# HiLab-git/FPL-plus

Hardware: AMD Instinct MI355X
Metric: 3D volumes/sec (train step, 80x160x160) (higher is better)
Workload: dtype bf16; 1 GPU; UNet3D-DSBN 32-base-ch bf16 (fp32 master weights), per-GPU batch 2x1x80x160x160 synthetic VS crops, DiceLoss + Adam, domain alternating per step; global_batch=2, parallelism=dp1, step=zero_grad+forward+loss+backward+allreduce+adam

## Files before the change

### fpl-plus_amd/csrc/common.h

```cpp
#pragma once
#include <hip/hip_runtime.h>
#include <math.h>
#include <stdint.h>
#include <stdio.h>
#include <stdarg.h>
#include <string.h>
#include "../../include/fplx.h"

typedef __bf16 bf16_t;

#define FPLX_WAVE 64

inline char* fplx_err_buf() {
  static thread_local char buf[512];
  return buf;
}
inline int fplx_fail(int code, const char* fmt, ...) {
  va_list ap;
  va_start(ap, fmt);
  vsnprintf(fplx_err_buf(), 512, fmt, ap);
  va_end(ap);
  return code;
}
inline int fplx_check_launch(const char* what) {
  hipError_t e = hipGetLastError();
  if (e != hipSuccess) return fplx_fail(FPLX_E_HIP, "%s: %s", what, hipGetErrorString(e));
  return FPLX_OK;
}
#define FPLX_REQUIRE(cond, code, ...) \
  do {                                 \
    if (!(cond)) return fplx_fail(code, __VA_ARGS__); \
  } while (0)

template <typename T> struct Act;
template <> struct Act<float> {
  static __device__ __forceinline__ float ld(const float* p) { return *p; }
  static __device__ __forceinline__ void st(float* p, float v) { *p = v; }
};
template <> struct Act<bf16_t> {
  static __device__ __forceinline__ float ld(const bf16_t* p) { return (float)*p; }
  static __device__ __forceinline__ void st(bf16_t* p, float v) { *p = (bf16_t)v; }
};

__device__ __forceinline__ float ld_dt(const void* p, int64_t i, int dt) {
  return dt == FPLX_F32 ? ((const float*)p)[i] : (float)((const bf16_t*)p)[i];
}
__device__ __forceinline__ void st_dt(void* p, int64_t i, int dt, float v) {
  if (dt == FPLX_F32) ((float*)p)[i] = v;
  else ((bf16_t*)p)[i] = (bf16_t)v;
}

__device__ __forceinline__ uint32_t key_nan_high(float f) {
  if (f != f) return 0xFFFFFFFFu;
  const uint32_t u = __float_as_uint(f);
  return (u & 0x80000000u) ? ~u : (u | 0x80000000u);
}
__device__ __forceinline__ uint32_t key_nan_low(float f) {
  if (f != f) return 0u;
  const uint32_t u = __float_as_uint(f);
  return (u & 0x80000000u) ? ~u : (u | 0x80000000u);
}
__device__ __forceinline__ float key_to_float(uint32_t k) {
  return __uint_as_float((k & 0x80000000u) ? (k & 0x7FFFFFFFu) : ~k);
}

__device__ __forceinline__ float wave_sum(float v) {
#pragma unroll
  for (int o = 32; o > 0; o >>= 1) v += __shfl_xor(v, o, 64);
  return v;
}
__device__ __forceinline__ double wave_sum_d(double v) {
#pragma unroll
  for (int o = 32; o > 0; o >>= 1) v += __shfl_xor(v, o, 64);
  return v;
}

#ifdef __HIPCC__
struct FplxOptimConst { float lr, wd, gscale, k0, k1, k2, k3, k4, k5; int first; };
__device__ __forceinline__ float fplx_optim_grad(float pi, float g, const FplxOptimConst& c) {
  return fmaf(c.wd, pi, g * c.gscale);
}
__device__ __forceinline__ void fplx_adam_elem(float& pi, float g, float& mi, float& vi, const FplxOptimConst& c) {
  const float gi = fplx_optim_grad(pi, g, c);
  mi = fmaf(c.k0, mi, c.k1 * gi);
  vi = fmaf(c.k3, vi, (c.k4 * gi) * gi);
  const float denom = fmaf(sqrtf(vi), c.k5, c.k2);
  pi = fmaf(-c.lr, mi / denom, pi);
}
template <bool MOM>
__device__ __forceinline__ void fplx_sgd_elem(float& pi, float g, float& buf, const FplxOptimConst& c) {
  const float gi = fplx_optim_grad(pi, g, c);
  if (MOM) {
    buf = fmaf(c.k0, buf, gi);
    pi = fmaf(-c.lr, buf, pi);
  } else {
    pi = fmaf(-c.lr, gi, pi);
  }
}
__device__ __forceinline__ void fplx_adadelta_elem(float& pi, float g, float& sq, float& acc, const FplxOptimConst& c) {
  const float gi = fplx_optim_grad(pi, g, c);
  sq = fmaf(c.k0, sq, (c.k1 * gi) * gi);
  const float stdv = sqrtf(sq + c.k2);
  const float ratio = sqrtf(acc + c.k2) / stdv;
  const float delta = ratio * gi;
  acc = fmaf(c.k0, acc, (c.k1 * delta) * delta);
  pi = fmaf(-c.lr, delta, pi);
}
__device__ __forceinline__ void fplx_adagrad_elem(float& pi, float g, float& sum, const FplxOptimConst& c) {
  const float gi = fplx_optim_grad(pi, g, c);
  sum = fmaf(gi, gi, sum);
  const float stdv = sqrtf(sum) + c.k2;
  pi = fmaf(-c.lr, gi / stdv, pi);
}
__device__ __forceinline__ void fplx_adamax_elem(float& pi, float g, float& mi, float& ui, const FplxOptimConst& c) {
  const float gi = fplx_optim_grad(pi, g, c);
  mi = fmaf(c.k0, mi, c.k1 * gi);
  const float decayed = c.k3 * ui;
  ui = fmaxf(decayed, fabsf(gi) + c.k2);
  pi = fmaf(-c.lr, mi / ui, pi);
}
__device__ __forceinline__ void fplx_asgd_elem(float& pi, float g, float& ax, const FplxOptimConst& c) {
  const float gi = fplx_optim_grad(pi, g, c);
  const float decayed = pi * c.k0;
  pi = fmaf(-c.lr, gi, decayed);
  const float d = pi - ax;
  ax = c.k3 == 1.f ? pi : fmaf(d, c.k3, ax);
}
template <bool MOM>
__device__ __forceinline__ void fplx_rmsprop_elem(float& pi, float g, float& sq, float& buf, const FplxOptimConst& c) {
  const float gi = fplx_optim_grad(pi, g, c);
  sq = fmaf(c.k0, sq, (c.k1 * gi) * gi);
  const float avg = sqrtf(sq) + c.k2;
  if (MOM) {
    buf = fmaf(c.k3, buf, gi / avg);
    pi = fmaf(-c.lr, buf, pi);
  } else {
    pi = fmaf(-c.lr, gi / avg, pi);
  }
}
__device__ __forceinline__ void fplx_rprop_elem(float& pi, float g, float& prev, float& ss, const FplxOptimConst& c) {
  float gi = g * c.gscale;
  if (c.first) { prev = 0.f; ss = c.lr; }
  const float s = gi * prev;
  const float f = s > 0.f ? c.k1 : (s < 0.f ? c.k0 : 1.f);
  const float scaled = ss * f;
  ss = fminf(fmaxf(scaled, c.k3), c.k4);
  if (s < 0.f) gi = 0.f;
  const float sg = gi > 0.f ? 1.f : (gi < 0.f ? -1.f : 0.f);
  pi = fmaf(-sg, ss, pi);
  prev = gi;
}
template <int KIND, int NS>
__device__ __forceinline__ void fplx_optim_elem(float& pi, float g, float& s0, float& s1, const FplxOptimConst& c) {
  if constexpr (KIND == FPLX_OPT_SGD) fplx_sgd_elem<NS == 1>(pi, g, s0, c);
  else if constexpr (KIND == FPLX_OPT_ADADELTA) fplx_adadelta_elem(pi, g, s0, s1, c);
  else if constexpr (KIND == FPLX_OPT_ADAGRAD) fplx_adagrad_elem(pi, g, s0, c);
  else if constexpr (KIND == FPLX_OPT_ADAMAX) fplx_adamax_elem(pi, g, s0, s1, c);
  else if constexpr (KIND == FPLX_OPT_ASGD) fplx_asgd_elem(pi, g, s0, c);
  else if constexpr (KIND == FPLX_OPT_RMSPROP) fplx_rmsprop_elem<NS == 2>(pi, g, s0, s1, c);
  else if constexpr (KIND == FPLX_OPT_ADAM) fplx_adam_elem(pi, g, s0, s1, c);
  else fplx_rprop_elem(pi, g, s0, s1, c);
}
#define FPLX_OPTIM_DISPATCH(kind, ns, X)                                       \
  switch ((kind) * 4 + (ns)) {                                                 \
    case FPLX_OPT_SGD * 4 + 0: X(FPLX_OPT_SGD, 0); break;                      \
    case FPLX_OPT_SGD * 4 + 1: X(FPLX_OPT_SGD, 1); break;                      \
    case FPLX_OPT_ADADELTA * 4 + 2: X(FPLX_OPT_ADADELTA, 2); break;            \
    case FPLX_OPT_ADAGRAD * 4 + 1: X(FPLX_OPT_ADAGRAD, 1); break;              \
    case FPLX_OPT_ADAMAX * 4 + 2: X(FPLX_OPT_ADAMAX, 2); break;                \
    case FPLX_OPT_ASGD * 4 + 1: X(FPLX_OPT_ASGD, 1); break;                    \
    case FPLX_OPT_RMSPROP * 4 + 1: X(FPLX_OPT_RMSPROP, 1); break;              \
    case FPLX_OPT_RMSPROP * 4 + 2: X(FPLX_OPT_RMSPROP, 2); break;              \
    case FPLX_OPT_ADAM * 4 + 2: X(FPLX_OPT_ADAM, 2); break;                    \
    default: X(FPLX_OPT_RPROP, 2); break;                                      \
  }
static inline int fplx_optim_consts(const char* who, int kind, const float* hp, int nhp, int step, float gscale, const void* s0,
                                    const void* s1, FplxOptimConst* c, int* ns) {
  static const int want[FPLX_OPT_COUNT] = {3, 4, 4, 5, 4, 5, 5, 5};
  FPLX_REQUIRE(kind >= 0 && kind < FPLX_OPT_COUNT, FPLX_E_BADSHAPE, "%s: unknown optimiser kind %d (0..%d)", who, kind,
               FPLX_OPT_COUNT - 1);
  FPLX_REQUIRE(hp, FPLX_E_NULL, "%s: null hyper-parameter array", who);
  FPLX_REQUIRE(nhp == want[kind], FPLX_E_BADSHAPE, "%s: kind %d takes %d hyper-parameters, got %d", who, kind, want[kind], nhp);
  FPLX_REQUIRE(step >= 1, FPLX_E_BADSHAPE, "%s: step=%d (1-based)", who, step);
  *c = {hp[0], 0.f, gscale, 0.f, 0.f, 0.f, 0.f, 0.f, 0.f, step == 1};
  int need = 2;
  switch (kind) {
    case FPLX_OPT_SGD:
      c->k0 = hp[1]; c->wd = hp[2];
      need = hp[1] != 0.f ? 1 : 0;
      break;
    case FPLX_OPT_ADADELTA:
      c->k0 = hp[1]; c->k1 = (float)(1.0 - (double)hp[1]); c->k2 = hp[2]; c->wd = hp[3];
      break;
    case FPLX_OPT_ADAGRAD:
      c->lr = (float)((double)hp[0] / (1.0 + (double)(step - 1) * (double)hp[1])); c->k2 = hp[2]; c->wd = hp[3];
      need = 1;
      break;
    case FPLX_OPT_ADAMAX:
      c->lr = (float)((double)hp[0] / (1.0 - pow((double)hp[1], step)));
      c->k0 = hp[1]; c->k1 = (float)(1.0 - (double)hp[1]); c->k3 = hp[2]; c->k2 = hp[3]; c->wd = hp[4];
      break;
    case FPLX_OPT_ASGD:
      c->k0 = (float)(1.0 - (double)hp[2] * (double)hp[0]); c->k3 = hp[1]; c->wd = hp[3];
      need = 1;
      break;
    case FPLX_OPT_RMSPROP:
      c->k0 = hp[1]; c->k1 = (float)(1.0 - (double)hp[1]); c->k2 = hp[2]; c->k3 = hp[3]; c->wd = hp[4];
      need = hp[3] > 0.f ? 2 : 1;
      break;
    case FPLX_OPT_ADAM:
      c->lr = (float)((double)hp[0] / (1.0 - pow((double)hp[1], step)));
      c->k0 = hp[1]; c->k1 = 1.f - hp[1]; c->k2 = hp[3]; c->k3 = hp[2]; c->k4 = 1.f - hp[2]; c->wd = hp[4];
      c->k5 = (float)(1.0 / sqrt(1.0 - pow((double)hp[2], step)));
      break;
    default:
      c->k0 = hp[1]; c->k1 = hp[2]; c->k3 = hp[3]; c->k4 = hp[4];
      break;
  }
  FPLX_REQUIRE((need < 1 || s0) && (need < 2 || s1), FPLX_E_NULL, "%s: kind %d needs %d state buffer(s) here", who, kind, need);
  *ns = need;
  return FPLX_OK;
}
struct FplxBlock { int x, y, z; };
__device__ __forceinline__ FplxBlock fplx_xcd_block(int on) {
  FplxBlock b = {(int)blockIdx.x, (int)blockIdx.y, (int)blockIdx.z};
  if (!on) return b;
  const unsigned gx = gridDim.x, gy = gridDim.y, gz = gridDim.z, t = gx * gy * gz;
  const unsigned l = (blockIdx.z * gy + blockIdx.y) * gx + blockIdx.x;
  const unsigned xcd = l & 7u, q = t >> 3, r = t & 7u;
  const unsigned lp = xcd * q + (xcd < r ? xcd : r) + (l >> 3);
  const unsigned per = gy * gz, xq = lp / per, rem = lp - xq * per;
  b.x = __builtin_amdgcn_readfirstlane((int)xq);
  b.z = __builtin_amdgcn_readfirstlane((int)(rem / gy));
  b.y = __builtin_amdgcn_readfirstlane((int)(rem % gy));
  return b;
}
struct FplxTileRange { int64_t first, end, step; };
__device__ __forceinline__ FplxTileRange fplx_xcd_tiles(int64_t ntiles, int on) {
  FplxTileRange t = {(int64_t)blockIdx.x, ntiles, (int64_t)gridDim.x};
  if (!on || gridDim.x < 16) return t;
  const unsigned c = blockIdx.x & 7u, xcd = (blockIdx.y * gridDim.x + blockIdx.x) & 7u;
  const int64_t q = ntiles >> 3, r = ntiles & 7;
  const int64_t start = xcd * q + ((int64_t)xcd < r ? xcd : r);
  t.first = start + (blockIdx.x >> 3);
  t.end = start + q + ((int64_t)xcd < r ? 1 : 0);
  t.step = (gridDim.x - c + 7u) >> 3;
  return t;
}
template <typename... P, typename... A>
inline void fplx_launch(void (*kernel)(P...), dim3 grid, dim3 block, size_t lds, hipStream_t st, A... args) {
  if (lds) (void)hipFuncSetAttribute((const void*)kernel, hipFuncAttributeMaxDynamicSharedMemorySize, (int)lds);
  kernel<<<grid, block, lds, st>>>(args...);
}
#endif
#define FPLX_KNOB_LIST(X)                                                                                              \
  X(XCD, "xcd", 1)                                                    \
  X(BRICK, "brick", 1)                                    \
  X(BRICK_FILL, "brick_fill", 192)           \
  X(BRICK_GEO, "brick_geo", -1)                    \
  X(BRICK_KSPLIT, "brick_ksplit", 0)                                             \
  X(EDGE_BLOCKS, "edge_blocks", 1024)                             \
  X(STEM_ROWS, "stem_rows", 1)                                              \
  X(OUTCONV_T, "outconv_t", 1)                                 \
  X(OUTCONV_DGRAD_MFMA, "outconv_dgrad_mfma", 1)                                                                       \
  X(OUTCONV_FWD_ROWS, "outconv_fwd_rows", 1)  \
  X(OUTCONV_DGRAD_ROWS, "outconv_dgrad_rows", 1)  \
  X(PACK_TILED, "pack_tiled", 1)                                                                                       \
  X(PACK_MULTI, "pack_multi", 1)                                                                                       \
  X(MARCH, "march", 1)                           \
  X(MARCH64_FW, "march64_fw", 0)                                \
  X(MARCH_DS, "march_ds", 0)                                       \
  X(MARCH128, "march128", 1)                                                                                           \
  X(MARCH64_LW, "march64_lw", 1)            \
  X(MARCH32_V2, "march32_v2", 4)              \
  X(WG_COT_MINVOX, "wg_cot_minvox", 0)                                                                                 \
  X(WG_TW, "wg_tw", 0)                                                                                                 \
  X(WG_CIT, "wg_cit", 2)                                                                                               \
  X(WG_COT, "wg_cot", 2)                                                                                               \
  X(WG_DS, "wg_ds", 0)                                                                                                 \
  X(WG_VOX, "wg_vox", 1)                              \
  X(WG_ROLL, "wg_roll", 1)                     \
  X(WG_ROLL_GEO, "wg_roll_geo", 0)          \
  X(WG_ROLL_M16, "wg_roll_m16", 1)                 \
  X(WG_ROLL_MB, "wg_roll_mb", 1)            \
  X(WG_ROLL_CUS, "wg_roll_cus", 256)                                \
  X(WG_ROLL_OVH, "wg_roll_ovh", 9)                     \
  X(WG_ROLL_MINVOX, "wg_roll_minvox", 0)                                                   \
  X(WG_ROLL2D, "wg_roll2d", 1)              \
  X(WG_ROLL2D_OVH, "wg_roll2d_ovh", 3)      \
  X(WG_REDUCE_ROWS, "wg_reduce_rows", 8)    \
  X(WG_VOX_LW, "wg_vox_lw", 1)              \
  X(WG_VOX_CUS, "wg_vox_cus", 128)          \
  X(WG_VOX_MAXV, "wg_vox_maxv", 10000)         \
  X(TILE_NT, "tile_nt", 0)                                                                                             \
  X(TILE_KS, "tile_ks", 0)                                                                                             \
  X(MID_TILE, "mid_tile", 1)                                                                                           \
  X(DECONV_ROWS, "deconv_rows", 1)                                                                                     \
  X(DECONV_DGRAD_ROWS, "deconv_dgrad_rows", 1)   \
  X(ROWS_SMALL_DIV, "rows_small_div", 16)   \
  X(EW_GROUP, "ew_group", 1)                                                                                           \
  X(POOL_COL, "pool_col", 1)                         \
  X(EW_INFLIGHT, "ew_inflight", 2)          \
  X(EW_INFLIGHT_REDUCE, "ew_inflight_reduce", 2)
enum FplxKnobId {
#define FPLX_KNOB_ENUM(id, key, def) FPLX_K_##id,
  FPLX_KNOB_LIST(FPLX_KNOB_ENUM)
#undef FPLX_KNOB_ENUM
  FPLX_K_COUNT
};
extern "C" __attribute__((visibility("hidden"))) int64_t fplx_knob_values[FPLX_K_COUNT];
static inline int64_t fplx_knob(int id) { return __atomic_load_n(&fplx_knob_values[id], __ATOMIC_RELAXED); }
static inline int fplx_xcd_on() { return (int)fplx_knob(FPLX_K_XCD); }

static inline int fplx_rows_for(int64_t voxels) {
  constexpr int cap = 512;
  const int div = voxels <= 32768 ? (int)fplx_knob(FPLX_K_ROWS_SMALL_DIV) : 64;
  int64_t r = (voxels + div - 1) / div;
  if (r > cap) r = cap;
  if (r < 1) r = 1;
  return (int)r;
}
```

### fpl-plus_amd/csrc/conv_march.hip

```cpp
#include "internal.h"
#include "gfx950.h"
#include <stdlib.h>
#include <type_traits>

namespace {

__device__ __attribute__((aligned(16))) const unsigned int fplx_zero16[4] = {0u, 0u, 0u, 0u};
#ifdef FPLX_STAMP
__device__ long long* fplx_stamp_buf;
#endif

struct MG {
  static constexpr int CIN = 32, ROWB = 64, CH = 4;
  static constexpr int FH = 16, FW = 32, SH = FH + 2, SW = FW + 2, SLAB = SH * SW;
  static constexpr int THREADS = 512;
  static constexpr int SLAB_CHUNKS = SLAB * CH, SLAB_DMA = (SLAB_CHUNKS + 63) / 64;
  static constexpr int SLAB_BYTES = SLAB_DMA * 1024, W_BYTES = 27 * 32 * ROWB;
  static constexpr int NPIECE = (SLAB_DMA + 7) / 8;
  static constexpr int STAGE_BYTES = 32 * 32 * 2;
  static constexpr int LDS = 2 * SLAB_BYTES + W_BYTES + 32 * 4 + NPIECE * THREADS * 4 + (THREADS / 64) * STAGE_BYTES;
  static __device__ __forceinline__ int swz(int row) { return (row >> 2) & 3; }
};

template <int MASK, class Side>
__device__ __forceinline__ void march_step(const char* __restrict__ sl, const char* __restrict__ wbuf, int wave, int r,
                                           int khalf, f32x16& A00, f32x16& A01, f32x16& A10, f32x16& A11, f32x16& A20,
                                           f32x16& A21, Side&& side) {
  bf16x8 fa[2][2], fb[2][3];
  const f32x16 zero = {0.f, 0.f, 0.f, 0.f, 0.f, 0.f, 0.f, 0.f, 0.f, 0.f, 0.f, 0.f, 0.f, 0.f, 0.f, 0.f};
  int vb = wave * 2 * MG::SW + r, rb = r;
  opaque_v(vb, rb);
  const char* wl0 = wbuf + rb * MG::ROWB + ((khalf ^ MG::swz(rb)) << 4);
  const char* wl1 = wbuf + rb * MG::ROWB + (((2 + khalf) ^ MG::swz(rb)) << 4);
  auto load_stage = [&](int q, int buf) {
    const int p = q >> 1, ks = q & 1;
    const int kh = p / 3, kw = p % 3;
    const int c = 2 * ks + khalf;
#pragma unroll
    for (int m = 0; m < 2; ++m) {
      const int vox = vb + (m + kh) * MG::SW + kw;
      fa[buf][m] = *reinterpret_cast<const bf16x8*>(sl + vox * MG::ROWB + ((c ^ MG::swz(vox)) << 4));
    }
#pragma unroll
    for (int kd = 0; kd < 3; ++kd)
      if ((MASK >> kd) & 1) fb[buf][kd] = *reinterpret_cast<const bf16x8*>((ks ? wl1 : wl0) + (kd * 9 + p) * 32 * MG::ROWB);
  };
  load_stage(0, 0);
#pragma unroll
  for (int q = 0; q < 18; ++q) {
    if (q + 1 < 18) load_stage(q + 1, (q + 1) & 1);
    __builtin_amdgcn_sched_barrier(0);
    const int b = q & 1;
    {
      if constexpr ((MASK & 1) != 0) A00 = __builtin_amdgcn_mfma_f32_32x32x16_bf16(fa[b][0], fb[b][0], q == 0 ? zero : A00, 0, 0, 0);
      if constexpr ((MASK & 2) != 0) A10 = __builtin_amdgcn_mfma_f32_32x32x16_bf16(fa[b][0], fb[b][1], A10, 0, 0, 0);
      if constexpr ((MASK & 4) != 0) A20 = __builtin_amdgcn_mfma_f32_32x32x16_bf16(fa[b][0], fb[b][2], A20, 0, 0, 0);
      if constexpr ((MASK & 1) != 0) A01 = __builtin_amdgcn_mfma_f32_32x32x16_bf16(fa[b][1], fb[b][0], q == 0 ? zero : A01, 0, 0, 0);
      if constexpr ((MASK & 2) != 0) A11 = __builtin_amdgcn_mfma_f32_32x32x16_bf16(fa[b][1], fb[b][1], A11, 0, 0, 0);
      if constexpr ((MASK & 4) != 0) A21 = __builtin_amdgcn_mfma_f32_32x32x16_bf16(fa[b][1], fb[b][2], A21, 0, 0, 0);
    }
    side(q);
    __builtin_amdgcn_sched_barrier(0);
  }
}

template <bool TWOD, bool ACT = false>
__global__ void __launch_bounds__(MG::THREADS)
conv_fwd_march32(const bf16_t* __restrict__ x, int64_t ldx, const bf16_t* __restrict__ wp,
                 const float* __restrict__ bias, bf16_t* __restrict__ y, int64_t ldy, int N, int D, int H, int W,
                 int Cout, float* __restrict__ stats, int tilesH, int tilesW, int dsegs, int dlen,
                 bf16_t* __restrict__ y1, int ysplit, int xcd, const float* __restrict__ slope_p = nullptr) {
  extern __shared__ __attribute__((aligned(16))) char smem[];
#ifdef FPLX_STAMP
  const long long st_launch = __builtin_amdgcn_s_memtime();
#endif
  char* slabs = smem;
  char* wbuf = smem + 2 * MG::SLAB_BYTES;
  float* bias_s = reinterpret_cast<float*>(wbuf + MG::W_BYTES);
  const int tid = threadIdx.x, lane = tid & 63;
  const int wave = __builtin_amdgcn_readfirstlane(tid >> 6);
  const int r = lane & 31, khalf = lane >> 5;
  const FplxBlock bid = fplx_xcd_block(xcd);
  int b = bid.x;
  const int seg = b % dsegs; b /= dsegs;
  const int tw = b % tilesW; b /= tilesW;
  const int th = b % tilesH; b /= tilesH;
  const int n = __builtin_amdgcn_readfirstlane(b);
  const int h0 = __builtin_amdgcn_readfirstlane(th * MG::FH), w0 = __builtin_amdgcn_readfirstlane(tw * MG::FW);
  const int d0 = __builtin_amdgcn_readfirstlane(seg * dlen);
  const int d1 = (d0 + dlen < D) ? d0 + dlen : D;
  const int n0 = bid.y * 32;

  constexpr int NPIECE = MG::NPIECE;
  int* soff_s = reinterpret_cast<int*>(bias_s + 32);
#pragma unroll
  for (int k = 0; k < NPIECE; ++k) {
    const int i = (wave + 8 * k) * 64 + lane;
    const int vox = i >> 2, c = (i & 3) ^ MG::swz(vox);
    const int hh = vox / MG::SW + h0 - 1, ww = vox % MG::SW + w0 - 1;
    const bool in = i < MG::SLAB_CHUNKS && hh >= 0 && hh < H && ww >= 0 && ww < W;
    soff_s[k * MG::THREADS + tid] = in ? (int)((((int64_t)hh * W + ww) * ldx + c * 8) * 2) : -1;
  }
  const int64_t xslice = (int64_t)H * W * ldx * 2;
  const char* xn = reinterpret_cast<const char*>(x) + (int64_t)n * D * xslice;
  auto slab_piece = [&](int s, int k, int so) {
    if (wave + 8 * k < MG::SLAB_DMA) {
      const char* xs = xn + s * xslice;
      const void* src = so >= 0 ? (const void*)(xs + (unsigned)so) : (const void*)fplx_zero16;
      lds_dma_global(src, lds_addr(slabs + ((s + 1) & 1) * MG::SLAB_BYTES + (wave + 8 * k) * 1024));
    }
  };

  f32x16 K0a, K0b, K1a, K1b, K2a, K2b, Ra, Rb;
#pragma unroll
  for (int i = 0; i < 16; ++i) K0a[i] = K0b[i] = K1a[i] = K1b[i] = K2a[i] = K2b[i] = Ra[i] = Rb[i] = 0.f;

  const int sbase = TWOD ? d0 : d0 - 1;
  if (sbase >= 0) {
#pragma unroll
    for (int k = 0; k < NPIECE; ++k) slab_piece(sbase, k, soff_s[k * MG::THREADS + tid]);
  }
  for (int j = wave; j < 27 * 32 * MG::CH / 64; j += 8) {
    const int i = j * 64 + lane;
    const int row = i >> 2, c = (i & 3) ^ MG::swz(row);
    lds_dma_global(wp + ((int64_t)(row >> 5) * Cout + n0 + (row & 31)) * MG::CIN + c * 8, lds_addr(wbuf + j * 1024));
  }
  if (tid < 32) bias_s[tid] = bias ? bias[n0 + tid] : 0.f;
  wait_vmcnt0();
  lds_barrier();

  const float bv = bias_s[r];
  float ssum = 0.f, qsum = 0.f;
  char* stg = reinterpret_cast<char*>(soff_s + NPIECE * MG::THREADS) + wave * MG::STAGE_BYTES;
  char* stg_w = stg + (4 * khalf) * 64 + r * 2;
  const char* stg_r = stg + lane * 16;
  unsigned wmask = 0;
#pragma unroll
  for (int i = 0; i < 16; ++i)
    if (w0 + (i & 3) + 8 * (i >> 2) + 4 * khalf < W) wmask |= 1u << i;
  const bool hok0 = h0 + wave * 2 < H, hok1 = h0 + wave * 2 + 1 < H;
  const unsigned ldy2 = (unsigned)ldy * 2u;
  bf16_t* ysel = bid.y >= ysplit ? y1 + (bid.y - ysplit) * 32 : y + n0;
  char* yn = reinterpret_cast<char*>(ysel) + (((int64_t)n * D * H + (h0 + wave * 2)) * W + w0) * ldy * 2;
  const int64_t yslice = (int64_t)H * W * ldy * 2;
  const unsigned soffb = (unsigned)(lane >> 2) * ldy2 + (unsigned)(lane & 3) * 16u;
  const bool sok0 = w0 + (lane >> 2) < W, sok1 = w0 + (lane >> 2) + 16 < W;
  const float slope_v = ACT ? *slope_p : 0.f;
  auto retire_elem = [&](f32x16& A, int m, int i) {
    const int wu = (i & 3) + 8 * (i >> 2);
    float ov = A[i] + bv;
    if (ACT) ov = ov > 0.f ? ov : ov * slope_v;
    *reinterpret_cast<bf16_t*>(stg_w + wu * 64) = (bf16_t)ov;
#ifndef FPLX_ABL_NOSTATS
    if (!ACT && (m ? hok1 : hok0) && ((wmask >> i) & 1u)) {
      ssum += ov;
      qsum = fmaf(ov, ov, qsum);
    }
#endif
  };
  auto retire_flush = [&](int m, int o) {
    if (m ? hok1 : hok0) {
      unsigned l2 = ldy2;
      opaque_s(l2);
      char* rowp = yn + o * yslice + (unsigned)(m * W) * l2;
      const u32x4 v0 = *reinterpret_cast<const u32x4*>(stg_r);
      const u32x4 v1 = *reinterpret_cast<const u32x4*>(stg_r + 1024);
      if (sok0) global_store_16(rowp + soffb, v0);
      if (sok1) global_store_16(rowp + 16u * l2 + soffb, v1);
    }
  };

  const int nd = d1 - d0;
  const int nsteps = TWOD ? nd + 1 : nd + 2;
#ifdef FPLX_STAMP
  long long st_step = 0, st_wait = 0, st_bar = 0;
  const long long st_begin = __builtin_amdgcn_s_memtime();
  const long long st_rbegin = __builtin_amdgcn_s_memrealtime();
#endif
  for (int t = 0; t < nsteps; ++t) {
#ifdef FPLX_STAMP
    const long long st0 = __builtin_amdgcn_s_memtime();
#endif
    const int s = sbase + t;
    const bool fetch = TWOD ? s + 1 < d1 : (s + 1 <= d1 && s + 1 < D);
    const bool wout = t >= (TWOD ? 2 : 3);
    const int o = s - 2;
    const char* sl = slabs + ((s + 1) & 1) * MG::SLAB_BYTES;
    int so[NPIECE];
#pragma unroll
    for (int k = 0; k < NPIECE; ++k) so[k] = soff_s[k * MG::THREADS + tid];
    auto side = [&](int q) {
#ifndef FPLX_ABL_NODMA
      if (q < NPIECE && fetch) slab_piece(s + 1, q, so[q < NPIECE ? q : 0]);
#endif
#ifdef FPLX_ABL_NORETIRE
      return;
#endif
      if (wout && q < 9) {
        if (q < 4) { retire_elem(Ra, 0, 4 * q); retire_elem(Ra, 0, 4 * q + 1); retire_elem(Ra, 0, 4 * q + 2); retire_elem(Ra, 0, 4 * q + 3); }
        if (q == 4) retire_flush(0, o);
        if (q >= 4 && q < 8) { retire_elem(Rb, 1, 4 * q - 16); retire_elem(Rb, 1, 4 * q - 15); retire_elem(Rb, 1, 4 * q - 14); retire_elem(Rb, 1, 4 * q - 13); }
        if (q == 8) retire_flush(1, o);
      }
    };
#define MARCH_STEP(MASK) march_step<MASK>(sl, wbuf, wave, r, khalf, K0a, K0b, K1a, K1b, K2a, K2b, side)
    if (TWOD ? t < nd : (s >= 0 && s < D)) {
      if constexpr (TWOD) {
        MARCH_STEP(2);
      } else {
        if (t == 0) MARCH_STEP(1);
        else if (t == 1) MARCH_STEP(3);
        else if (t < nd) MARCH_STEP(7);
        else if (t == nd) MARCH_STEP(6);
        else MARCH_STEP(4);
      }
    } else {
#pragma unroll
      for (int q = 0; q < 9; ++q) side(q);
#pragma unroll
      for (int i = 0; i < 16; ++i) K0a[i] = K0b[i] = 0.f;
    }
#undef MARCH_STEP
    Ra = K2a; Rb = K2b; K2a = K1a; K2b = K1b; K1a = K0a; K1b = K0b;
#ifdef FPLX_STAMP
    const long long st1 = __builtin_amdgcn_s_memtime();
#endif
    wait_vmcnt0();
#ifdef FPLX_STAMP
    const long long st2 = __builtin_amdgcn_s_memtime();
#endif
    lds_barrier();
#ifdef FPLX_STAMP
    const long long st3 = __builtin_amdgcn_s_memtime();
    st_step += st1 - st0; st_wait += st2 - st1; st_bar += st3 - st2;
#endif
  }
#ifdef FPLX_STAMP
  if (lane == 0) {
    long long* o = fplx_stamp_buf + ((int64_t)(blockIdx.y * gridDim.x + blockIdx.x) * 8 + wave) * 6;
    o[0] = st_step; o[1] = st_wait; o[2] = st_bar; o[3] = __builtin_amdgcn_s_memtime() - st_begin; o[4] = nsteps;
    o[5] = __builtin_amdgcn_s_memrealtime() - st_rbegin;
  }
#endif
  {
#pragma unroll
    for (int i = 0; i < 16; ++i) retire_elem(Ra, 0, i);
    retire_flush(0, d1 - 1);
#pragma unroll
    for (int i = 0; i < 16; ++i) retire_elem(Rb, 1, i);
    retire_flush(1, d1 - 1);
  }

  if (stats) {
    lds_barrier();
    float* red = reinterpret_cast<float*>(smem);
    const float a = ssum + __shfl_xor(ssum, 32, 64), q2 = qsum + __shfl_xor(qsum, 32, 64);
    if (lane < 32) { red[(wave * 2 + 0) * 32 + r] = a; red[(wave * 2 + 1) * 32 + r] = q2; }
    lds_barrier();
    if (tid < 64) {
      const int which = tid >> 5, c = tid & 31;
      float t = 0.f;
#pragma unroll
      for (int wv = 0; wv < 8; ++wv) t += red[(wv * 2 + which) * 32 + c];
      stats[((int64_t)bid.x * 2 + which) * Cout + n0 + c] = t;
    }
  }
}

struct MG2 {
  static constexpr int CIN = 32, ROWB = 64, CH = 4;
  static constexpr int FH = 16, FW = 32, SH = FH + 2, SW = FW + 2, SLAB = SH * SW;
  static constexpr int THREADS = 256, WAVES = 4;
  static constexpr int SLAB_CHUNKS = SLAB * CH, SLAB_DMA = (SLAB_CHUNKS + 63) / 64;
  static constexpr int SLAB_BYTES = SLAB_DMA * 1024, W_BYTES = 27 * 32 * ROWB;
  static constexpr int NPIECE = (SLAB_DMA + WAVES - 1) / WAVES;
  static constexpr int STAGE_BYTES = 32 * 32 * 2;
  static constexpr int LDS = 2 * SLAB_BYTES + W_BYTES + 32 * 4 + WAVES * 2 * STAGE_BYTES + NPIECE * THREADS * 4;
  static __device__ __forceinline__ int swz(int row) { return (row >> 2) & 3; }
};

template <bool STATS>
__global__ void __launch_bounds__(MG2::THREADS)
conv_fwd_march32v2(const bf16_t* __restrict__ x, int64_t ldx, const bf16_t* __restrict__ wp,
                   const float* __restrict__ bias, bf16_t* __restrict__ y, int64_t ldy, int N, int D, int H, int W,
                   int Cout, float* __restrict__ stats, int tilesH, int tilesW, int dsegs, int dlen,
                   bf16_t* __restrict__ y1, int ysplit, int xcd) {
  using G = MG2;
  extern __shared__ __attribute__((aligned(16))) char smem[];
  char* slabs = smem;
  char* wbuf = smem + 2 * G::SLAB_BYTES;
  float* bias_s = reinterpret_cast<float*>(wbuf + G::W_BYTES);
  const int tid = threadIdx.x, lane = tid & 63;
  const int wave = __builtin_amdgcn_readfirstlane(tid >> 6);
  const int r = lane & 31, khalf = lane >> 5;
  const FplxBlock bid = fplx_xcd_block(xcd);
  int b = bid.x;
  const int seg = b % dsegs; b /= dsegs;
  const int tw = b % tilesW; b /= tilesW;
  const int th = b % tilesH; b /= tilesH;
  const int n = __builtin_amdgcn_readfirstlane(b);
  const int h0 = __builtin_amdgcn_readfirstlane(th * G::FH), w0 = __builtin_amdgcn_readfirstlane(tw * G::FW);
  const int d0 = __builtin_amdgcn_readfirstlane(seg * dlen);
  const int d1 = (d0 + dlen < D) ? d0 + dlen : D;
  const int n0 = bid.y * 32;

  constexpr int NPIECE = G::NPIECE;
  unsigned* voff_s = reinterpret_cast<unsigned*>(smem + 2 * G::SLAB_BYTES + G::W_BYTES + 32 * 4 + G::WAVES * 2 * G::STAGE_BYTES);
#pragma unroll
  for (int k = 0; k < NPIECE; ++k) {
    int piece = wave + G::WAVES * k;
    if (piece > G::SLAB_DMA - 1) piece = G::SLAB_DMA - 1;
    const int i = piece * 64 + lane;
    const int vox = i >> 2, c = (i & 3) ^ G::swz(vox);
    const int hh = vox / G::SW + h0 - 1, ww = vox % G::SW + w0 - 1;
    const bool in = i < G::SLAB_CHUNKS && hh >= 0 && hh < H && ww >= 0 && ww < W;
    voff_s[k * G::THREADS + tid] = in ? (unsigned)((((int64_t)hh * W + ww) * ldx + c * 8) * 2) : 0x40000000u;
  }
  const int64_t xslice = (int64_t)H * W * ldx * 2;
  const char* xn = reinterpret_cast<const char*>(x) + (int64_t)n * D * xslice;
  u32x4 rsrc;
  rsrc[0] = __builtin_amdgcn_readfirstlane((unsigned)(size_t)xn);
  rsrc[1] = __builtin_amdgcn_readfirstlane((unsigned)((size_t)xn >> 32) & 0xFFFFu);
  rsrc[2] = __builtin_amdgcn_readfirstlane((unsigned)((int64_t)D * xslice));
  rsrc[3] = 0x00020000u;
  const unsigned xslice32 = __builtin_amdgcn_readfirstlane((unsigned)xslice);
  auto slab_piece = [&](int s, int k, unsigned vo) {
    int piece = wave + G::WAVES * k;
    if (piece > G::SLAB_DMA - 1) piece = G::SLAB_DMA - 1;
    const unsigned dst = lds_addr(slabs + ((s + 1) & 1) * G::SLAB_BYTES + piece * 1024);
    const unsigned so = __builtin_amdgcn_readfirstlane((s >= 0 && s < D) ? (unsigned)s * xslice32 : 0x40000000u);
    lds_dma_buffer(rsrc, vo, so, dst);
  };

  f32x16 S[4][4];
#pragma unroll
  for (int a = 0; a < 4; ++a)
#pragma unroll
    for (int m = 0; m < 4; ++m)
#pragma unroll
      for (int i = 0; i < 16; ++i) S[a][m][i] = 0.f;

  __syncthreads();
  const int sbase = d0 - 1;
#pragma unroll
  for (int k = 0; k < NPIECE; ++k) slab_piece(sbase, k, voff_s[k * G::THREADS + tid]);
  for (int j = wave; j < 27 * 32 * G::CH / 64; j += G::WAVES) {
    const int i = j * 64 + lane;
    const int row = i >> 2, c = (i & 3) ^ G::swz(row);
    lds_dma_global(wp + ((int64_t)(row >> 5) * Cout + n0 + (row & 31)) * G::CIN + c * 8, lds_addr(wbuf + j * 1024));
  }
  if (tid < 32) bias_s[tid] = bias ? bias[n0 + tid] : 0.f;
  wait_vmcnt0();
  lds_barrier();

  const float bv = bias_s[r];
  float ssum = 0.f, qsum = 0.f;
  char* stg = reinterpret_cast<char*>(bias_s + 32) + wave * 2 * G::STAGE_BYTES;
  const unsigned ldy2 = (unsigned)ldy * 2u;
  bf16_t* ysel = bid.y >= ysplit ? y1 + (bid.y - ysplit) * 32 : y + n0;
  char* yn = reinterpret_cast<char*>(ysel) + (((int64_t)n * D * H + (h0 + wave * 4)) * W + w0) * ldy * 2;
  const int64_t yslice = (int64_t)H * W * ldy * 2;
  const unsigned soffb = (unsigned)(lane >> 2) * ldy2 + (unsigned)(lane & 3) * 16u;
  auto retire_elems = [&](const f32x16& A, int m, int i0, int cnt) {
    char* w_ = stg + (m & 1) * G::STAGE_BYTES + (4 * khalf) * 64 + r * 2;
#pragma unroll
    for (int i = i0; i < i0 + cnt; ++i) {
      const int wu = (i & 3) + 8 * (i >> 2);
      const float ov = A[i] + bv;
      *reinterpret_cast<bf16_t*>(w_ + wu * 64) = (bf16_t)ov;
      if (STATS) { ssum += ov; qsum = fmaf(ov, ov, qsum); }
    }
  };
  auto retire_flush = [&](int m, int o) {
    const char* r_ = stg + (m & 1) * G::STAGE_BYTES + lane * 16;
    unsigned l2 = ldy2;
    opaque_s(l2);
    char* rowp = yn + o * yslice + (unsigned)(m * W) * l2;
    const u32x4 v0 = *reinterpret_cast<const u32x4*>(r_);
    const u32x4 v1 = *reinterpret_cast<const u32x4*>(r_ + 1024);
    global_store_16(rowp + soffb, v0);
    global_store_16(rowp + 16u * l2 + soffb, v1);
  };

  const int nd = d1 - d0;
  const int nsteps = nd + 2;
  const f32x16 zero = {0.f, 0.f, 0.f, 0.f, 0.f, 0.f, 0.f, 0.f, 0.f, 0.f, 0.f, 0.f, 0.f, 0.f, 0.f, 0.f};

  bf16x8 fa[2][6], fb[9];
  auto load_a = [&](const char* sl, int g, int buf) {
    const int kw = g >> 1, ks = g & 1, c = 2 * ks + khalf;
    int vb = wave * 4 * G::SW + r;
    opaque_v(vb);
#pragma unroll
    for (int rho = 0; rho < 6; ++rho) {
      const int vox = vb + rho * G::SW + kw;
      fa[buf][rho] = *reinterpret_cast<const bf16x8*>(sl + vox * G::ROWB + ((c ^ G::swz(vox)) << 4));
    }
  };
  auto load_b = [&](int g, int kd) {
    const int kw = g >> 1, ks = g & 1;
    int rb = r;
    opaque_v(rb);
    const char* wl = wbuf + rb * G::ROWB + (((2 * ks + khalf) ^ G::swz(rb)) << 4);
#pragma unroll
    for (int kh = 0; kh < 3; ++kh)
      fb[kd * 3 + kh] = *reinterpret_cast<const bf16x8*>(wl + ((kd * 9 + kh * 3 + kw) * 32) * G::ROWB);
  };
  load_a(slabs + ((sbase + 1) & 1) * G::SLAB_BYTES, 0, 0);
  load_b(0, 0); load_b(0, 1); load_b(0, 2);
  auto step = [&](auto rot_c, int t) {
    constexpr int ROT = decltype(rot_c)::value;
    const int s = sbase + t;
    const int o = (s - 2 > d0) ? s - 2 : d0;
    const char* sl = slabs + ((s + 1) & 1) * G::SLAB_BYTES;
    const char* sl_next = slabs + (s & 1) * G::SLAB_BYTES;
    const bool on0 = t < nd, on1 = t >= 1 && t <= nd, on2 = t >= 2;
    f32x16 (&K0)[4] = S[(0 - ROT) & 3];
    f32x16 (&K1)[4] = S[(1 - ROT) & 3];
    f32x16 (&K2)[4] = S[(2 - ROT) & 3];
    f32x16 (&R)[4] = S[(3 - ROT) & 3];
    u32x4 fl0, fl1;
    unsigned vo0 = 0, vo1 = 0, vo2 = 0;
#pragma unroll
    for (int g = 0; g < 6; ++g) {
      const int bf = g & 1;
      const int p0 = g < 2 ? 3 * g : 2 * g + 2, np = g < 2 ? 3 : (g < 4 ? 2 : 0);
      if (np > 0) {
        vo0 = voff_s[p0 * G::THREADS + tid];
        vo1 = voff_s[(p0 + 1) * G::THREADS + tid];
        if (np > 2) vo2 = voff_s[(p0 + 2) * G::THREADS + tid];
      }
      if (g >= 1 && g <= 4) {
        const char* r_ = stg + ((g - 1) & 1) * G::STAGE_BYTES + lane * 16;
        fl0 = *reinterpret_cast<const u32x4*>(r_);
        fl1 = *reinterpret_cast<const u32x4*>(r_ + 1024);
      }
      if (g < 4) retire_elems(R[g], g, 0, 8);
      if (on0) {
#pragma unroll
        for (int m = 0; m < 4; ++m)
#pragma unroll
          for (int kh = 0; kh < 3; ++kh)
            K0[m] = __builtin_amdgcn_mfma_f32_32x32x16_bf16(fa[bf][m + kh], fb[0 + kh], (g == 0 && kh == 0) ? zero : K0[m], 0, 0, 0);
      }
      __builtin_amdgcn_sched_barrier(0);
      if (g < 5) load_a(sl, g + 1, bf ^ 1); else load_a(sl_next, 0, 0);
      load_b((g + 1) % 6, 0);
      if (g >= 1 && g <= 4) {
        unsigned l2 = ldy2;
        opaque_s(l2);
        char* rowp = yn + o * yslice + (unsigned)((g - 1) * W) * l2;
        global_store_16(rowp + soffb, fl0);
        global_store_16(rowp + 16u * l2 + soffb, fl1);
      }
      if (np > 0) {
        slab_piece(s + 1, p0, vo0);
        slab_piece(s + 1, p0 + 1, vo1);
        if (np > 2) slab_piece(s + 1, p0 + 2, vo2);
      }
      if (on1) {
#pragma unroll
        for (int m = 0; m < 4; ++m)
#pragma unroll
          for (int kh = 0; kh < 3; ++kh)
            K1[m] = __builtin_amdgcn_mfma_f32_32x32x16_bf16(fa[bf][m + kh], fb[3 + kh], K1[m], 0, 0, 0);
      }
      __builtin_amdgcn_sched_barrier(0);
      load_b((g + 1) % 6, 1);
      if (g < 4) retire_elems(R[g], g, 8, 8);
      if (on2) {
#pragma unroll
        for (int m = 0; m < 4; ++m)
#pragma unroll
          for (int kh = 0; kh < 3; ++kh)
            K2[m] = __builtin_amdgcn_mfma_f32_32x32x16_bf16(fa[bf][m + kh], fb[6 + kh], K2[m], 0, 0, 0);
      }
      load_b((g + 1) % 6, 2);
      __builtin_amdgcn_sched_barrier(0);
      if (g == 4) {
        wait_vmcnt0();
        lds_barrier();
      }
    }
  };
  using C0 = std::integral_constant<int, 0>;
  using C1 = std::integral_constant<int, 1>;
  using C2 = std::integral_constant<int, 2>;
  using C3 = std::integral_constant<int, 3>;
#ifdef FPLX_STAMP
  const long long st_begin = __builtin_amdgcn_s_memtime();
  const long long st_rbegin = __builtin_amdgcn_s_memrealtime();
#endif
  int t = 0;
  for (;;) {
    step(C0{}, t); ++t;
    if (t >= nsteps) break;
    step(C1{}, t); ++t;
    if (t >= nsteps) break;
    step(C2{}, t); ++t;
    if (t >= nsteps) break;
    if (STATS && t == 3) { ssum = 0.f; qsum = 0.f; }
    step(C3{}, t); ++t;
    if (t >= nsteps) break;
  }
#ifdef FPLX_STAMP
  if (lane == 0) {
    long long* o_ = fplx_stamp_buf + ((int64_t)(blockIdx.y * gridDim.x + blockIdx.x) * 8 + wave) * 6;
    o_[0] = 0; o_[1] = 0; o_[2] = 0; o_[3] = __builtin_amdgcn_s_memtime() - st_begin; o_[4] = nsteps;
    o_[5] = __builtin_amdgcn_s_memrealtime() - st_rbegin;
  }
#endif
  auto drain = [&](auto rot_c) {
    constexpr int ROT = decltype(rot_c)::value;
    f32x16 (&R)[4] = S[(3 - ROT) & 3];
#pragma unroll
    for (int m = 0; m < 4; ++m) { retire_elems(R[m], m, 0, 16); retire_flush(m, d1 - 1); }
  };
  switch (nsteps & 3) {
    case 0: drain(C0{}); break;
    case 1: drain(C1{}); break;
    case 2: drain(C2{}); break;
    default: drain(C3{}); break;
  }

  if (STATS && stats) {
    lds_barrier();
    float* red = reinterpret_cast<float*>(smem);
    const float a = ssum + __shfl_xor(ssum, 32, 64), q2 = qsum + __shfl_xor(qsum, 32, 64);
    if (lane < 32) { red[(wave * 2 + 0) * 32 + r] = a; red[(wave * 2 + 1) * 32 + r] = q2; }
    lds_barrier();
    if (tid < 64) {
      const int which = tid >> 5, c = tid & 31;
      float tt = 0.f;
#pragma unroll
      for (int wv = 0; wv < 4; ++wv) tt += red[(wv * 2 + which) * 32 + c];
      stats[((int64_t)bid.x * 2 + which) * Cout + n0 + c] = tt;
    }
  }
}

template <bool STATS, int ASWZ, bool ACT = false>
__global__ void __launch_bounds__(MG2::THREADS)
conv_fwd_march32v3(const bf16_t* __restrict__ x, int64_t ldx, const bf16_t* __restrict__ wp,
                   const float* __restrict__ bias, bf16_t* __restrict__ y, int64_t ldy, int N, int D, int H, int W,
                   int Cout, float* __restrict__ stats, int tilesH, int tilesW, int dsegs, int dlen,
                   bf16_t* __restrict__ y1, int ysplit, int xcd, const float* __restrict__ slope_p = nullptr) {
  using G = MG2;
  extern __shared__ __attribute__((aligned(16))) char smem[];
  char* slabs = smem;
  char* wbuf = smem + 2 * G::SLAB_BYTES;
  float* bias_s = reinterpret_cast<float*>(wbuf + G::W_BYTES);
  const int tid = threadIdx.x, lane = tid & 63;
  const int wave = __builtin_amdgcn_readfirstlane(tid >> 6);
  const int r16 = lane & 15, kg = lane >> 4;
  const FplxBlock bid = fplx_xcd_block(xcd);
  int b = bid.x;
  const int seg = b % dsegs; b /= dsegs;
  const int tw = b % tilesW; b /= tilesW;
  const int th = b % tilesH; b /= tilesH;
  const int n = __builtin_amdgcn_readfirstlane(b);
  const int h0 = __builtin_amdgcn_readfirstlane(th * G::FH), w0 = __builtin_amdgcn_readfirstlane(tw * G::FW);
  const int d0 = __builtin_amdgcn_readfirstlane(seg * dlen);
  const int d1 = (d0 + dlen < D) ? d0 + dlen : D;
  const int n0 = bid.y * 32;

  auto wswz = [](int row) { const int q = (row >> 2) & 3; return (4 - q) & 3; };
  auto aswz = [](int vox) { return ASWZ ? ((vox >> 2) & 1) << 1 : (vox >> 2) & 3; };
  constexpr int NPIECE = G::NPIECE;
  unsigned* voff_s = reinterpret_cast<unsigned*>(smem + 2 * G::SLAB_BYTES + G::W_BYTES + 32 * 4 + G::WAVES * 2 * G::STAGE_BYTES);
#pragma unroll
  for (int k = 0; k < NPIECE; ++k) {
    int piece = wave + G::WAVES * k;
    if (piece > G::SLAB_DMA - 1) piece = G::SLAB_DMA - 1;
    const int i = piece * 64 + lane;
    const int vox = i >> 2, c = (i & 3) ^ aswz(vox);
    const int hh = vox / G::SW + h0 - 1, ww = vox % G::SW + w0 - 1;
    const bool in = i < G::SLAB_CHUNKS && hh >= 0 && hh < H && ww >= 0 && ww < W;
    voff_s[k * G::THREADS + tid] = in ? (unsigned)((((int64_t)hh * W + ww) * ldx + c * 8) * 2) : 0x40000000u;
  }
  const int64_t xslice = (int64_t)H * W * ldx * 2;
  const char* xn = reinterpret_cast<const char*>(x) + (int64_t)n * D * xslice;
  u32x4 rsrc;
  rsrc[0] = __builtin_amdgcn_readfirstlane((unsigned)(size_t)xn);
  rsrc[1] = __builtin_amdgcn_readfirstlane((unsigned)((size_t)xn >> 32) & 0xFFFFu);
  rsrc[2] = __builtin_amdgcn_readfirstlane((unsigned)((int64_t)D * xslice));
  rsrc[3] = 0x00020000u;
  const unsigned xslice32 = __builtin_amdgcn_readfirstlane((unsigned)xslice);
  auto slab_piece = [&](int s, int k, unsigned vo) {
    int piece = wave + G::WAVES * k;
    if (piece > G::SLAB_DMA - 1) piece = G::SLAB_DMA - 1;
    const unsigned dst = lds_addr(slabs + ((s + 1) & 1) * G::SLAB_BYTES + piece * 1024);
    const unsigned so = __builtin_amdgcn_readfirstlane((s >= 0 && s < D) ? (unsigned)s * xslice32 : 0x40000000u);
    lds_dma_buffer(rsrc, vo, so, dst);
  };

  f32x4 S[4][4][4];
#pragma unroll
  for (int a = 0; a < 4; ++a)
#pragma unroll
    for (int m = 0; m < 4; ++m)
#pragma unroll
      for (int q = 0; q < 4; ++q)
#pragma unroll
        for (int i = 0; i < 4; ++i) S[a][m][q][i] = 0.f;

  __syncthreads();
  const int sbase = d0 - 1;
#pragma unroll
  for (int k = 0; k < NPIECE; ++k) slab_piece(sbase, k, voff_s[k * G::THREADS + tid]);
  for (int j = wave; j < 27 * 32 * G::CH / 64; j += G::WAVES) {
    const int i = j * 64 + lane;
    const int row = i >> 2, c = (i & 3) ^ wswz(row);
    lds_dma_global(wp + ((int64_t)(row >> 5) * Cout + n0 + (row & 31)) * G::CIN + c * 8, lds_addr(wbuf + j * 1024));
  }
  if (tid < 32) bias_s[tid] = bias ? bias[n0 + tid] : 0.f;
  wait_vmcnt0();
  lds_barrier();

  const float bv0 = bias_s[r16], bv1 = bias_s[16 + r16];
  float ssum0 = 0.f, qsum0 = 0.f, ssum1 = 0.f, qsum1 = 0.f;
  char* stg = reinterpret_cast<char*>(bias_s + 32) + wave * 2 * G::STAGE_BYTES;
  const unsigned ldy2 = (unsigned)ldy * 2u;
  bf16_t* ysel = bid.y >= ysplit ? y1 + (bid.y - ysplit) * 32 : y + n0;
  char* yn = reinterpret_cast<char*>(ysel) + (((int64_t)n * D * H + (h0 + wave * 4)) * W + w0) * ldy * 2;
  const int64_t yslice = (int64_t)H * W * ldy * 2;
  const unsigned soffb = (unsigned)(lane >> 2) * ldy2 + (unsigned)(lane & 3) * 16u;
  const float slope_v = ACT ? *slope_p : 0.f;
  auto retire_half = [&](const f32x4 (&A)[4], int m, int mh) {
    char* w_ = stg + (m & 1) * G::STAGE_BYTES + (mh * 16 + 4 * kg) * 64 + r16 * 2;
#pragma unroll
    for (int i = 0; i < 4; ++i) {
      float o0 = A[mh * 2 + 0][i] + bv0, o1 = A[mh * 2 + 1][i] + bv1;
      if (ACT) { o0 = o0 > 0.f ? o0 : o0 * slope_v; o1 = o1 > 0.f ? o1 : o1 * slope_v; }
      *reinterpret_cast<bf16_t*>(w_ + i * 64) = (bf16_t)o0;
      *reinterpret_cast<bf16_t*>(w_ + i * 64 + 32) = (bf16_t)o1;
      if (STATS) { ssum0 += o0; qsum0 = fmaf(o0, o0, qsum0); ssum1 += o1; qsum1 = fmaf(o1, o1, qsum1); }
    }
  };
  auto retire_flush = [&](int m, int o) {
    const char* r_ = stg + (m & 1) * G::STAGE_BYTES + lane * 16;
    unsigned l2 = ldy2;
    opaque_s(l2);
    char* rowp = yn + o * yslice + (unsigned)(m * W) * l2;
    const u32x4 v0 = *reinterpret_cast<const u32x4*>(r_);
    const u32x4 v1 = *reinterpret_cast<const u32x4*>(r_ + 1024);
    global_store_16(rowp + soffb, v0);
    global_store_16(rowp + 16u * l2 + soffb, v1);
  };

  const int nd = d1 - d0;
  const int nsteps = nd + 2;
  const f32x4 zero = {0.f, 0.f, 0.f, 0.f};

  bf16x8 fa[2][6], fb[18];
  auto load_a = [&](const char* sl, int g, int buf) {
    const int kw = g >> 1, mh = g & 1;
    int vb = wave * 4 * G::SW + r16;
    opaque_v(vb);
#pragma unroll
    for (int rho = 0; rho < 6; ++rho) {
      const int vox = vb + rho * G::SW + kw + mh * 16;
      fa[buf][rho] = *reinterpret_cast<const bf16x8*>(sl + vox * G::ROWB + ((kg ^ aswz(vox)) << 4));
    }
  };
  auto load_b = [&](int kw, int kd) {
    int rb = r16;
    opaque_v(rb);
    const char* wl = wbuf + rb * G::ROWB + ((kg ^ wswz(rb)) << 4);
#pragma unroll
    for (int kh = 0; kh < 3; ++kh)
#pragma unroll
      for (int nh = 0; nh < 2; ++nh)
        fb[kd * 6 + kh * 2 + nh] = *reinterpret_cast<const bf16x8*>(wl + (((kd * 9 + kh * 3 + kw) * 32) + nh * 16) * G::ROWB);
  };
  load_a(slabs + ((sbase + 1) & 1) * G::SLAB_BYTES, 0, 0);
  load_b(0, 0); load_b(0, 1); load_b(0, 2);
  auto step = [&](auto rot_c, int t) {
    constexpr int ROT = decltype(rot_c)::value;
    const int s = sbase + t;
    const int o = (s - 2 > d0) ? s - 2 : d0;
    const char* sl = slabs + ((s + 1) & 1) * G::SLAB_BYTES;
    const char* sl_next = slabs + (s & 1) * G::SLAB_BYTES;
    const bool on0 = t < nd, on1 = t >= 1 && t <= nd, on2 = t >= 2;
    f32x4 (&K0)[4][4] = S[(0 - ROT) & 3];
    f32x4 (&K1)[4][4] = S[(1 - ROT) & 3];
    f32x4 (&K2)[4][4] = S[(2 - ROT) & 3];
    f32x4 (&R)[4][4] = S[(3 - ROT) & 3];
    u32x4 fl0, fl1;
    unsigned vo0 = 0, vo1 = 0, vo2 = 0;
#pragma unroll
    for (int g = 0; g < 6; ++g) {
      const int bf = g & 1, kw = g >> 1, mh = g & 1;
      const int p0 = g < 2 ? 3 * g : 2 * g + 2, np = g < 2 ? 3 : (g < 4 ? 2 : 0);
      if (np > 0) {
        vo0 = voff_s[p0 * G::THREADS + tid];
        vo1 = voff_s[(p0 + 1) * G::THREADS + tid];
        if (np > 2) vo2 = voff_s[(p0 + 2) * G::THREADS + tid];
      }
      if (g >= 1 && g <= 4) {
        const char* r_ = stg + ((g - 1) & 1) * G::STAGE_BYTES + lane * 16;
        fl0 = *reinterpret_cast<const u32x4*>(r_);
        fl1 = *reinterpret_cast<const u32x4*>(r_ + 1024);
      }
      if (g < 4) retire_half(R[g], g, 0);
      if (on0) {
#pragma unroll
        for (int m = 0; m < 4; ++m)
#pragma unroll
          for (int kh = 0; kh < 3; ++kh)
#pragma unroll
            for (int nh = 0; nh < 2; ++nh)
              K0[m][mh * 2 + nh] = __builtin_amdgcn_mfma_f32_16x16x32_bf16(fa[bf][m + kh], fb[0 + kh * 2 + nh],
                                                                          (kw == 0 && kh == 0) ? zero : K0[m][mh * 2 + nh], 0, 0, 0);
      }
      __builtin_amdgcn_sched_barrier(0);
      if (g < 5) load_a(sl, g + 1, bf ^ 1); else load_a(sl_next, 0, 0);
      if (mh == 1) load_b((kw + 1) % 3, 0);
      if (g >= 1 && g <= 4) {
        unsigned l2 = ldy2;
        opaque_s(l2);
        char* rowp = yn + o * yslice + (unsigned)((g - 1) * W) * l2;
        global_store_16(rowp + soffb, fl0);
        global_store_16(rowp + 16u * l2 + soffb, fl1);
      }
      if (np > 0) {
        slab_piece(s + 1, p0, vo0);
        slab_piece(s + 1, p0 + 1, vo1);
        if (np > 2) slab_piece(s + 1, p0 + 2, vo2);
      }
      if (on1) {
#pragma unroll
        for (int m = 0; m < 4; ++m)
#pragma unroll
          for (int kh = 0; kh < 3; ++kh)
#pragma unroll
            for (int nh = 0; nh < 2; ++nh)
              K1[m][mh * 2 + nh] = __builtin_amdgcn_mfma_f32_16x16x32_bf16(fa[bf][m + kh], fb[6 + kh * 2 + nh], K1[m][mh * 2 + nh], 0, 0, 0);
      }
      __builtin_amdgcn_sched_barrier(0);
      if (mh == 1) load_b((kw + 1) % 3, 1);
      if (g < 4) retire_half(R[g], g, 1);
      if (on2) {
#pragma unroll
        for (int m = 0; m < 4; ++m)
#pragma unroll
          for (int kh = 0; kh < 3; ++kh)
#pragma unroll
            for (int nh = 0; nh < 2; ++nh)
              K2[m][mh * 2 + nh] = __builtin_amdgcn_mfma_f32_16x16x32_bf16(fa[bf][m + kh], fb[12 + kh * 2 + nh], K2[m][mh * 2 + nh], 0, 0, 0);
      }
      if (mh == 1) load_b((kw + 1) % 3, 2);
      __builtin_amdgcn_sched_barrier(0);
      if (g == 4) {
        wait_vmcnt0();
        lds_barrier();
      }
    }
  };
  using C0 = std::integral_constant<int, 0>;
  using C1 = std::integral_constant<int, 1>;
  using C2 = std::integral_constant<int, 2>;
  using C3 = std::integral_constant<int, 3>;
#ifdef FPLX_STAMP
  const long long st_begin = __builtin_amdgcn_s_memtime();
  const long long st_rbegin = __builtin_amdgcn_s_memrealtime();
#endif
  int t = 0;
  for (;;) {
    step(C0{}, t); ++t;
    if (t >= nsteps) break;
    step(C1{}, t); ++t;
    if (t >= nsteps) break;
    step(C2{}, t); ++t;
    if (t >= nsteps) break;
    if (STATS && t == 3) { ssum0 = qsum0 = ssum1 = qsum1 = 0.f; }
    step(C3{}, t); ++t;
    if (t >= nsteps) break;
  }
#ifdef FPLX_STAMP
  if (lane == 0) {
    long long* o_ = fplx_stamp_buf + ((int64_t)(blockIdx.y * gridDim.x + blockIdx.x) * 8 + wave) * 6;
    o_[0] = 0; o_[1] = 0; o_[2] = 0; o_[3] = __builtin_amdgcn_s_memtime() - st_begin; o_[4] = nsteps;
    o_[5] = __builtin_amdgcn_s_memrealtime() - st_rbegin;
  }
#endif
  auto drain = [&](auto rot_c) {
    constexpr int ROT = decltype(rot_c)::value;
    f32x4 (&R)[4][4] = S[(3 - ROT) & 3];
#pragma unroll
    for (int m = 0; m < 4; ++m) { retire_half(R[m], m, 0); retire_half(R[m], m, 1); retire_flush(m, d1 - 1); }
  };
  switch (nsteps & 3) {
    case 0: drain(C0{}); break;
    case 1: drain(C1{}); break;
    case 2: drain(C2{}); break;
    default: drain(C3{}); break;
  }

  if (STATS && stats) {
    lds_barrier();
    float* red = reinterpret_cast<float*>(smem);
    float a0 = ssum0, a1 = ssum1, q0 = qsum0, q1 = qsum1;
    a0 += __shfl_xor(a0, 16, 64); a0 += __shfl_xor(a0, 32, 64);
    a1 += __shfl_xor(a1, 16, 64); a1 += __shfl_xor(a1, 32, 64);
    q0 += __shfl_xor(q0, 16, 64); q0 += __shfl_xor(q0, 32, 64);
    q1 += __shfl_xor(q1, 16, 64); q1 += __shfl_xor(q1, 32, 64);
    if (lane < 16) {
      red[(wave * 2 + 0) * 32 + r16] = a0; red[(wave * 2 + 0) * 32 + 16 + r16] = a1;
      red[(wave * 2 + 1) * 32 + r16] = q0; red[(wave * 2 + 1) * 32 + 16 + r16] = q1;
    }
    lds_barrier();
    if (tid < 64) {
      const int which = tid >> 5, c = tid & 31;
      float tt = 0.f;
#pragma unroll
      for (int wv = 0; wv < 4; ++wv) tt += red[(wv * 2 + which) * 32 + c];
      stats[((int64_t)bid.x * 2 + which) * Cout + n0 + c] = tt;
    }
  }
}

template <int FWV>
struct MG64T {
  static constexpr int ROWB = 64, CH = 4;
  static constexpr int FW = FWV, FH = 256 / FWV, SH = FH + 2, SW = FW + 2, SLAB = SH * SW;
  static constexpr int HPM = 32 / FW;
  static constexpr int THREADS = 256;
  static constexpr int SLAB_CHUNKS = SLAB * CH, SLAB_DMA = (SLAB_CHUNKS + 63) / 64;
  static constexpr int SLAB_BYTES = SLAB * ROWB, WH_BYTES = 27 * 32 * ROWB;
  static constexpr int NPIECE = (SLAB_DMA + 3) / 4;
  static constexpr int STAGE_BYTES = 32 * 32 * 2;
  static constexpr int LDS = 2 * SLAB_BYTES + 2 * WH_BYTES + 32 * 4 + (THREADS / 64) * STAGE_BYTES;
  static __device__ __forceinline__ int swz(int row) { return (row >> 2) & 3; }
};
using MG64 = MG64T<32>;

template <int MASK, bool FIRST, class G, class Side>
__device__ __forceinline__ void march64_half(const char* __restrict__ sl, const char* __restrict__ wh, int wave, int r,
                                             int khalf, f32x16& A00, f32x16& A01, f32x16& A10, f32x16& A11,
                                             f32x16& A20, f32x16& A21, Side&& side) {
  bf16x8 fa[2][2], fb[2][3];
  const f32x16 zero = {0.f, 0.f, 0.f, 0.f, 0.f, 0.f, 0.f, 0.f, 0.f, 0.f, 0.f, 0.f, 0.f, 0.f, 0.f, 0.f};
  int vb = (wave * 2 * G::HPM + r / G::FW) * G::SW + r % G::FW, rb = r;
  opaque_v(vb, rb);
  const char* wl0 = wh + rb * G::ROWB + ((khalf ^ G::swz(rb)) << 4);
  const char* wl1 = wh + rb * G::ROWB + (((2 + khalf) ^ G::swz(rb)) << 4);
  auto load_a = [&](int q, int m) {
    const int p = q >> 1, ks = q & 1, kh = p / 3, kw = p % 3, c = 2 * ks + khalf;
    const int vox = vb + (m * G::HPM + kh) * G::SW + kw;
    return *reinterpret_cast<const bf16x8*>(sl + vox * G::ROWB + ((c ^ G::swz(vox)) << 4));
  };
  auto load_b = [&](int q, int kd) {
    const int p = q >> 1, ks = q & 1;
    return *reinterpret_cast<const bf16x8*>((ks ? wl1 : wl0) + (kd * 9 + p) * 32 * G::ROWB);
  };
  fa[0][0] = load_a(0, 0); fa[0][1] = load_a(0, 1);
#pragma unroll
  for (int kd = 0; kd < 3; ++kd)
    if ((MASK >> kd) & 1) fb[0][kd] = load_b(0, kd);
#pragma unroll
  for (int q = 0; q < 18; ++q) {
    const int b = q & 1, nb = b ^ 1;
#define M64_GAP(G, LOADSTMT, MFMASTMT)                                                                              \
    if (q + 1 < 18) { LOADSTMT; }                                                                                   \
    side(q, G);                                                                                                     \
    __builtin_amdgcn_sched_barrier(0);                                                                              \
    MFMASTMT;                                                                                                       \
    __builtin_amdgcn_sched_barrier(0);
    M64_GAP(0, fa[nb][0] = load_a(q + 1, 0),
            if constexpr ((MASK & 1) != 0) A00 = __builtin_amdgcn_mfma_f32_32x32x16_bf16(fa[b][0], fb[b][0], (FIRST && q == 0) ? zero : A00, 0, 0, 0))
    M64_GAP(1, fa[nb][1] = load_a(q + 1, 1),
            if constexpr ((MASK & 2) != 0) A10 = __builtin_amdgcn_mfma_f32_32x32x16_bf16(fa[b][0], fb[b][1], A10, 0, 0, 0))
    M64_GAP(2, if constexpr ((MASK & 1) != 0) fb[nb][0] = load_b(q + 1, 0),
            if constexpr ((MASK & 4) != 0) A20 = __builtin_amdgcn_mfma_f32_32x32x16_bf16(fa[b][0], fb[b][2], A20, 0, 0, 0))
    M64_GAP(3, if constexpr ((MASK & 2) != 0) fb[nb][1] = load_b(q + 1, 1),
            if constexpr ((MASK & 1) != 0) A01 = __builtin_amdgcn_mfma_f32_32x32x16_bf16(fa[b][1], fb[b][0], (FIRST && q == 0) ? zero : A01, 0, 0, 0))
    M64_GAP(4, if constexpr ((MASK & 4) != 0) fb[nb][2] = load_b(q + 1, 2),
            if constexpr ((MASK & 2) != 0) A11 = __builtin_amdgcn_mfma_f32_32x32x16_bf16(fa[b][1], fb[b][1], A11, 0, 0, 0))
    M64_GAP(5, (void)0,
            if constexpr ((MASK & 4) != 0) A21 = __builtin_amdgcn_mfma_f32_32x32x16_bf16(fa[b][1], fb[b][2], A21, 0, 0, 0))
#undef M64_GAP
  }
}

template <class G, bool TWOD, int NQ, bool ACT = false>
__global__ void __launch_bounds__(256)
conv_fwd_march64(const bf16_t* __restrict__ x, int64_t ldx, const bf16_t* __restrict__ wp,
                 const float* __restrict__ bias, bf16_t* __restrict__ y, int64_t ldy, int N, int D, int H, int W,
                 int Cout, float* __restrict__ stats, int tilesH, int tilesW, int dsegs, int dlen,
                 const bf16_t* __restrict__ x1, int xcd, const float* __restrict__ slope_p = nullptr, int nmod0 = 0) {
  extern __shared__ __attribute__((aligned(16))) char smem[];
  char* slabs = smem;
  char* wbuf = smem + 2 * G::SLAB_BYTES;
  float* bias_s = reinterpret_cast<float*>(wbuf + 2 * G::WH_BYTES);
  const int tid = threadIdx.x, lane = tid & 63;
  const int wave = __builtin_amdgcn_readfirstlane(tid >> 6);
  const int r = lane & 31, khalf = lane >> 5;
  const FplxBlock bid = fplx_xcd_block(xcd);
  int b = bid.x;
  const int seg = b % dsegs; b /= dsegs;
  const int tw = b % tilesW; b /= tilesW;
  const int th = b % tilesH; b /= tilesH;
  const int n = __builtin_amdgcn_readfirstlane(b);
  const int h0 = __builtin_amdgcn_readfirstlane(th * G::FH), w0 = __builtin_amdgcn_readfirstlane(tw * G::FW);
  const int d0 = __builtin_amdgcn_readfirstlane(seg * dlen);
  const int d1 = (d0 + dlen < D) ? d0 + dlen : D;
  const int n0 = bid.y * 32;

  constexpr int NPIECE = G::NPIECE;
  int soff[NPIECE];
#pragma unroll
  for (int k = 0; k < NPIECE; ++k) {
    const int i = (wave + 4 * k) * 64 + lane;
    const int vox = i >> 2, c = (i & 3) ^ G::swz(vox);
    const int hh = vox / G::SW + h0 - 1, ww = vox % G::SW + w0 - 1;
    const bool in = hh >= 0 && hh < H && ww >= 0 && ww < W;
    soff[k] = i >= G::SLAB_CHUNKS ? -2 : (in ? (int)((((int64_t)hh * W + ww) * ldx + c * 8) * 2) : -1);
  }
  const int64_t xslice = (int64_t)H * W * ldx * 2;
  const char* xn = reinterpret_cast<const char*>(x) + (int64_t)(nmod0 > 0 ? n % nmod0 : n) * D * xslice;
  const char* xn1 = reinterpret_cast<const char*>(x1 ? x1 : x + 32) + (int64_t)n * D * xslice;
  auto slab_piece = [&](int s, int hf, int k) {
    if (wave + 4 * k < G::SLAB_DMA && soff[k] != -2) {
      const char* xs = (NQ == 2 ? (hf ? xn1 : xn) : xn + hf * 64) + s * xslice;
      const void* src = soff[k] >= 0 ? (const void*)(xs + (unsigned)soff[k]) : (const void*)fplx_zero16;
      lds_dma_global(src, lds_addr(slabs + (hf & 1) * G::SLAB_BYTES + (wave + 4 * k) * 1024));
    }
  };
  constexpr int CIN = NQ * 32;
  const char* wlane = reinterpret_cast<const char*>(wp) + ((int64_t)(n0 + (lane >> 2)) * CIN) * 2 +
                      (((lane & 3) ^ ((lane >> 4) & 3)) << 4);
  auto w_piece = [&](int qt, int j) {
    const int64_t row0 = (int64_t)(j >> 1) * Cout + (j & 1) * 16;
    lds_dma_global(wlane + row0 * (CIN * 2) + qt * 64, lds_addr(wbuf + (qt & 1) * G::WH_BYTES + j * 1024));
  };

  f32x16 K0a, K0b, K1a, K1b, K2a, K2b, Ra, Rb;
#pragma unroll
  for (int i = 0; i < 16; ++i) K0a[i] = K0b[i] = K1a[i] = K1b[i] = K2a[i] = K2b[i] = Ra[i] = Rb[i] = 0.f;

  const int sbase = TWOD ? d0 : d0 - 1;
  if (sbase >= 0) {
#pragma unroll
    for (int k = 0; k < NPIECE; ++k) { slab_piece(sbase, 0, k); }
  }
  if constexpr (NQ == 2) {
    for (int j = wave; j < 2 * 27 * 32 * G::CH / 64; j += 4) {
      const int i = j * 64 + lane;
      const int hf = i / (27 * 32 * G::CH), ii = i % (27 * 32 * G::CH);
      const int row = ii >> 2, c = (ii & 3) ^ G::swz(row);
      lds_dma_global(wp + ((int64_t)(row >> 5) * Cout + n0 + (row & 31)) * 64 + hf * 32 + c * 8, lds_addr(wbuf + j * 1024));
    }
  } else {
    for (int j = wave; j < 54; j += 4) w_piece(0, j);
  }
  if (tid < 32) bias_s[tid] = bias ? bias[n0 + tid] : 0.f;
  wait_vmcnt0();
  lds_barrier();

  const float bv = bias_s[r];
  float ssum = 0.f, qsum = 0.f;
  char* stg = reinterpret_cast<char*>(bias_s + 32) + wave * G::STAGE_BYTES;
  char* stg_w = stg + (4 * khalf) * 64 + r * 2;
  const char* stg_r = stg + lane * 16;
  const int hb = h0 + wave * 2 * G::HPM;
  unsigned wmask0 = 0, wmask1 = 0;
#pragma unroll
  for (int i = 0; i < 16; ++i) {
    const int mr = (i & 3) + 8 * (i >> 2) + 4 * khalf;
    if (w0 + mr % G::FW < W) {
      if (hb + mr / G::FW < H) wmask0 |= 1u << i;
      if (hb + G::HPM + mr / G::FW < H) wmask1 |= 1u << i;
    }
  }
  const unsigned ldy2 = (unsigned)ldy * 2u;
  char* yn = reinterpret_cast<char*>(y) + ((((int64_t)n * D * H + hb) * W + w0) * ldy + n0) * 2;
  const int64_t yslice = (int64_t)H * W * ldy * 2;
  const unsigned soffb = (unsigned)(lane >> 2) * ldy2 + (unsigned)(lane & 3) * 16u;
  const unsigned step1 = G::FW == 32 ? 16u : (unsigned)W;
  const bool wok = w0 + (lane >> 2) < W;
  bool sok[2][2];
#pragma unroll
  for (int m = 0; m < 2; ++m) {
    sok[m][0] = wok && hb + m * G::HPM < H;
    sok[m][1] = G::FW == 32 ? (sok[m][0] && w0 + (lane >> 2) + 16 < W) : (wok && hb + m * G::HPM + 1 < H);
  }
  const float slope_v = ACT ? *slope_p : 0.f;
  auto retire_elem = [&](f32x16& A, int m, int i) {
    const int wu = (i & 3) + 8 * (i >> 2);
    float ov = A[i] + bv;
    if (ACT) ov = ov > 0.f ? ov : ov * slope_v;
    *reinterpret_cast<bf16_t*>(stg_w + wu * 64) = (bf16_t)ov;
    if (!ACT && (((m ? wmask1 : wmask0) >> i) & 1u)) {
      ssum += ov;
      qsum = fmaf(ov, ov, qsum);
    }
  };
  auto retire_flush = [&](int m, int o) {
    if (sok[m][0] || sok[m][1]) {
      unsigned l2 = ldy2;
      opaque_s(l2);
      char* rowp = yn + o * yslice + (unsigned)(m * G::HPM * W) * l2;
      const u32x4 v0 = *reinterpret_cast<const u32x4*>(stg_r);
      const u32x4 v1 = *reinterpret_cast<const u32x4*>(stg_r + 1024);
      if (sok[m][0]) global_store_16(rowp + soffb, v0);
      if (sok[m][1]) global_store_16(rowp + step1 * l2 + soffb, v1);
    }
  };

  const int nd = d1 - d0;
  const int nsteps = TWOD ? nd + 1 : nd + 2;
  for (int t = 0; t < nsteps; ++t) {
    const int s = sbase + t;
    const bool live = TWOD ? t < nd : (s >= 0 && s < D);
    const bool wout = t >= (TWOD ? 2 : 3);
    const int o = s - 2;
#pragma unroll
    for (int hf = 0; hf < NQ; ++hf) {
      const int ns = hf < NQ - 1 ? s : s + 1, nh = (hf + 1) % NQ;
      const bool fetch = hf < NQ - 1 ? live : (TWOD ? ns < d1 : (ns >= 0 && ns < D && ns <= d1));
      const bool wfetch = NQ > 2 && !(t == nsteps - 1 && hf == NQ - 1);
      auto side = [&](int q, int g) {
        if (g == 5 && q < NPIECE && fetch) slab_piece(ns, nh, q < NPIECE ? q : 0);
        if constexpr (NQ > 2) {
          if (g == 4 && q != 3 && q != 7 && wfetch) {
            const int j = (TWOD ? 18 : 0) + wave + 4 * (q - (q > 3) - (q > 7));
            if (j < (TWOD ? 36 : 54)) w_piece(nh, j);
          }
        }
        if (hf == 0 && wout && q < 8) {
          if (g < 4) {
            if (q < 4) retire_elem(Ra, 0, 4 * q + g);
            else retire_elem(Rb, 1, 4 * (q - 4) + g);
          }
          if (g == 4 && q == 3) retire_flush(0, o);
          if (g == 4 && q == 7) retire_flush(1, o);
        }
      };
      const char* sl = slabs + (hf & 1) * G::SLAB_BYTES;
      const char* wh = wbuf + (hf & 1) * G::WH_BYTES;
#define M64_STEP(MASK)                                                                                              \
  do {                                                                                                              \
    if (hf == 0) march64_half<MASK, true, G>(sl, wh, wave, r, khalf, K0a, K0b, K1a, K1b, K2a, K2b, side);           \
    else march64_half<MASK, false, G>(sl, wh, wave, r, khalf, K0a, K0b, K1a, K1b, K2a, K2b, side);                  \
  } while (0)
      if (live) {
        if constexpr (TWOD) {
          M64_STEP(2);
        } else {
          if (t == 0) M64_STEP(1);
          else if (t == 1) M64_STEP(3);
          else if (t < nd) M64_STEP(7);
          else if (t == nd) M64_STEP(6);
          else M64_STEP(4);
        }
      } else {
#pragma unroll
        for (int q = 0; q < 8; ++q)
#pragma unroll
          for (int g = 0; g < 6; ++g) side(q, g);
        if (hf == 0) {
#pragma unroll
          for (int i = 0; i < 16; ++i) K0a[i] = K0b[i] = 0.f;
        }
      }
#undef M64_STEP
      wait_vmcnt0();
      lds_barrier();
    }
    Ra = K2a; Rb = K2b; K2a = K1a; K2b = K1b; K1a = K0a; K1b = K0b;
  }
#pragma unroll
  for (int i = 0; i < 16; ++i) retire_elem(Ra, 0, i);
  retire_flush(0, d1 - 1);
#pragma unroll
  for (int i = 0; i < 16; ++i) retire_elem(Rb, 1, i);
  retire_flush(1, d1 - 1);

  if (stats) {
    lds_barrier();
    float* red = reinterpret_cast<float*>(smem);
    const float a = ssum + __shfl_xor(ssum, 32, 64), q2 = qsum + __shfl_xor(qsum, 32, 64);
    if (lane < 32) { red[(wave * 2 + 0) * 32 + r] = a; red[(wave * 2 + 1) * 32 + r] = q2; }
    lds_barrier();
    if (tid < 64) {
      const int which = tid >> 5, c = tid & 31;
      float tt = 0.f;
#pragma unroll
      for (int wv = 0; wv < 4; ++wv) tt += red[(wv * 2 + which) * 32 + c];
      stats[((int64_t)bid.x * 2 + which) * Cout + n0 + c] = tt;
    }
  }
}

template <class G, bool TWOD, int NQ, bool ACT = false>
__global__ void __launch_bounds__(512)
conv_fwd_march64_lw(const bf16_t* __restrict__ x, int64_t ldx, const bf16_t* __restrict__ wp,
                    const float* __restrict__ bias, bf16_t* __restrict__ y, int64_t ldy, int N, int D, int H, int W,
                    int Cout, float* __restrict__ stats, int tilesH, int tilesW, int dsegs, int dlen,
                    const bf16_t* __restrict__ x1, int xcd, const float* __restrict__ slope_p = nullptr, int nmod0 = 0) {
  extern __shared__ __attribute__((aligned(16))) char smem[];
  char* slabs = smem;
  char* wbuf = smem + 2 * G::SLAB_BYTES;
  float* bias_s = reinterpret_cast<float*>(wbuf + 2 * G::WH_BYTES);
  const int tid = threadIdx.x, lane = tid & 63;
  const int wave8 = __builtin_amdgcn_readfirstlane(tid >> 6);
  const bool loader = wave8 >= 4;
  const int wave = wave8 & 3;
  const int r = lane & 31, khalf = lane >> 5;
  const FplxBlock bid = fplx_xcd_block(xcd);
  int b = bid.x;
  const int seg = b % dsegs; b /= dsegs;
  const int tw = b % tilesW; b /= tilesW;
  const int th = b % tilesH; b /= tilesH;
  const int n = __builtin_amdgcn_readfirstlane(b);
  const int h0 = __builtin_amdgcn_readfirstlane(th * G::FH), w0 = __builtin_amdgcn_readfirstlane(tw * G::FW);
  const int d0 = __builtin_amdgcn_readfirstlane(seg * dlen);
  const int d1 = (d0 + dlen < D) ? d0 + dlen : D;
  const int n0 = bid.y * 32;
  constexpr int CIN = NQ * 32;
  const int sbase = TWOD ? d0 : d0 - 1;
  const int nd = d1 - d0;
  const int nsteps = TWOD ? nd + 1 : nd + 2;
  if constexpr (NQ == 2) {
    for (int j = wave8; j < 2 * 27 * 32 * G::CH / 64; j += 8) {
      const int i = j * 64 + lane;
      const int hf = i / (27 * 32 * G::CH), ii = i % (27 * 32 * G::CH);
      const int row = ii >> 2, c = (ii & 3) ^ G::swz(row);
      lds_dma_global(wp + ((int64_t)(row >> 5) * Cout + n0 + (row & 31)) * 64 + hf * 32 + c * 8, lds_addr(wbuf + j * 1024));
    }
  }
  const char* wlane = reinterpret_cast<const char*>(wp) + ((int64_t)(n0 + (lane >> 2)) * CIN) * 2 +
                      (((lane & 3) ^ ((lane >> 4) & 3)) << 4);
  auto w_piece = [&](int qt, int j) {
    const int64_t row0 = (int64_t)(j >> 1) * Cout + (j & 1) * 16;
    lds_dma_global(wlane + row0 * (CIN * 2) + qt * 64, lds_addr(wbuf + (qt & 1) * G::WH_BYTES + j * 1024));
  };
  if constexpr (NQ != 2) {
    for (int j = wave8; j < 54; j += 8) w_piece(0, j);
  }
  if (tid < 32) bias_s[tid] = bias ? bias[n0 + tid] : 0.f;

  if (loader) {
    constexpr int NPIECE = G::NPIECE;
    unsigned soff[NPIECE];
#pragma unroll
    for (int k = 0; k < NPIECE; ++k) {
      const int i = (wave + 4 * k) * 64 + lane;
      const int vox = i >> 2, c = (i & 3) ^ G::swz(vox);
      const int hh = vox / G::SW + h0 - 1, ww = vox % G::SW + w0 - 1;
      const bool in = hh >= 0 && hh < H && ww >= 0 && ww < W;
      soff[k] = i >= G::SLAB_CHUNKS ? 0xFFFFFFFFu : (in ? (unsigned)((((int64_t)hh * W + ww) * ldx + c * 8) * 2) : 0x40000000u);
    }
    const int64_t xslice = (int64_t)H * W * ldx * 2;
    const char* xn = reinterpret_cast<const char*>(x) + (int64_t)(nmod0 > 0 ? n % nmod0 : n) * D * xslice;
    const char* xn1 = reinterpret_cast<const char*>(x1 ? x1 : x + 32) + (int64_t)n * D * xslice;
    const unsigned lds0 = lds_addr(smem);
    auto slab_part = [&](int s_, int hf) {
      const char* xs = (NQ == 2 ? (hf ? xn1 : xn) : xn + hf * 64) + s_ * xslice;
      const u32x4 rx = buffer_rsrc(xs, xslice);
#pragma unroll
      for (int k = 0; k < NPIECE; ++k)
        if (wave + 4 * k < G::SLAB_DMA && soff[k] != 0xFFFFFFFFu)
          lds_dma_buffer(rx, soff[k], 0u, lds0 + (unsigned)((hf & 1) * G::SLAB_BYTES + (wave + 4 * k) * 1024));
    };
    if (sbase >= 0) slab_part(sbase, 0);
    wait_vmcnt0();
    lds_barrier();
    for (int t = 0; t < nsteps; ++t) {
      const int s = sbase + t;
      const bool live = TWOD ? t < nd : (s >= 0 && s < D);
#pragma unroll
      for (int hf = 0; hf < NQ; ++hf) {
        const int ns = hf < NQ - 1 ? s : s + 1, nh = (hf + 1) % NQ;
        const bool fetch = hf < NQ - 1 ? live : (TWOD ? ns < d1 : (ns >= 0 && ns < D && ns <= d1));
        const bool wfetch = NQ > 2 && !(t == nsteps - 1 && hf == NQ - 1);
        if (fetch) slab_part(ns, nh);
        if constexpr (NQ > 2) {
          if (wfetch)
            for (int j = (TWOD ? 18 : 0) + wave; j < (TWOD ? 36 : 54); j += 4) w_piece(nh, j);
        }
        wait_vmcnt0();
        lds_barrier();
      }
    }
    if (stats) { lds_barrier(); lds_barrier(); }
    return;
  }

  f32x16 K0a, K0b, K1a, K1b, K2a, K2b, Ra, Rb;
#pragma unroll
  for (int i = 0; i < 16; ++i) K0a[i] = K0b[i] = K1a[i] = K1b[i] = K2a[i] = K2b[i] = Ra[i] = Rb[i] = 0.f;
  wait_vmcnt0();
  lds_barrier();

  const float bv = bias_s[r];
  float ssum = 0.f, qsum = 0.f;
  char* stg = reinterpret_cast<char*>(bias_s + 32) + wave * G::STAGE_BYTES;
  char* stg_w = stg + (4 * khalf) * 64 + r * 2;
  const char* stg_r = stg + lane * 16;
  const int hb = h0 + wave * 2 * G::HPM;
  unsigned wmask0 = 0, wmask1 = 0;
#pragma unroll
  for (int i = 0; i < 16; ++i) {
    const int mr = (i & 3) + 8 * (i >> 2) + 4 * khalf;
    if (w0 + mr % G::FW < W) {
      if (hb + mr / G::FW < H) wmask0 |= 1u << i;
      if (hb + G::HPM + mr / G::FW < H) wmask1 |= 1u << i;
    }
  }
  const unsigned ldy2 = (unsigned)ldy * 2u;
  char* yn = reinterpret_cast<char*>(y) + ((((int64_t)n * D * H + hb) * W + w0) * ldy + n0) * 2;
  const int64_t yslice = (int64_t)H * W * ldy * 2;
  const unsigned soffb = (unsigned)(lane >> 2) * ldy2 + (unsigned)(lane & 3) * 16u;
  const unsigned step1 = G::FW == 32 ? 16u : (unsigned)W;
  const bool wok = w0 + (lane >> 2) < W;
  bool sok[2][2];
#pragma unroll
  for (int m = 0; m < 2; ++m) {
    sok[m][0] = wok && hb + m * G::HPM < H;
    sok[m][1] = G::FW == 32 ? (sok[m][0] && w0 + (lane >> 2) + 16 < W) : (wok && hb + m * G::HPM + 1 < H);
  }
  const float slope_v = ACT ? *slope_p : 0.f;
  auto retire_elem = [&](f32x16& A, int m, int i) {
    const int wu = (i & 3) + 8 * (i >> 2);
    float ov = A[i] + bv;
    if (ACT) ov = ov > 0.f ? ov : ov * slope_v;
    *reinterpret_cast<bf16_t*>(stg_w + wu * 64) = (bf16_t)ov;
    if (!ACT && (((m ? wmask1 : wmask0) >> i) & 1u)) {
      ssum += ov;
      qsum = fmaf(ov, ov, qsum);
    }
  };
  auto retire_flush = [&](int m, int o) {
    if (sok[m][0] || sok[m][1]) {
      unsigned l2 = ldy2;
      opaque_s(l2);
      char* rowp = yn + o * yslice + (unsigned)(m * G::HPM * W) * l2;
      const u32x4 v0 = *reinterpret_cast<const u32x4*>(stg_r);
      const u32x4 v1 = *reinterpret_cast<const u32x4*>(stg_r + 1024);
      if (sok[m][0]) global_store_16(rowp + soffb, v0);
      if (sok[m][1]) global_store_16(rowp + step1 * l2 + soffb, v1);
    }
  };
  for (int t = 0; t < nsteps; ++t) {
    const int s = sbase + t;
    const bool live = TWOD ? t < nd : (s >= 0 && s < D);
    const bool wout = t >= (TWOD ? 2 : 3);
    const int o = s - 2;
#pragma unroll
    for (int hf = 0; hf < NQ; ++hf) {
      auto side = [&](int q, int g) {
        if (hf == 0 && wout && q < 8) {
          if (g < 4) {
            if (q < 4) retire_elem(Ra, 0, 4 * q + g);
            else retire_elem(Rb, 1, 4 * (q - 4) + g);
          }
          if (g == 4 && q == 3) retire_flush(0, o);
          if (g == 4 && q == 7) retire_flush(1, o);
        }
      };
      const char* sl = slabs + (hf & 1) * G::SLAB_BYTES;
      const char* wh = wbuf + (hf & 1) * G::WH_BYTES;
#define M64_STEP(MASK)                                                                                              \
  do {                                                                                                              \
    if (hf == 0) march64_half<MASK, true, G>(sl, wh, wave, r, khalf, K0a, K0b, K1a, K1b, K2a, K2b, side);           \
    else march64_half<MASK, false, G>(sl, wh, wave, r, khalf, K0a, K0b, K1a, K1b, K2a, K2b, side);                  \
  } while (0)
      if (live) {
        if constexpr (TWOD) {
          M64_STEP(2);
        } else {
          if (t == 0) M64_STEP(1);
          else if (t == 1) M64_STEP(3);
          else if (t < nd) M64_STEP(7);
          else if (t == nd) M64_STEP(6);
          else M64_STEP(4);
        }
      } else {
#pragma unroll
        for (int q = 0; q < 8; ++q)
#pragma unroll
          for (int g = 0; g < 6; ++g) side(q, g);
        if (hf == 0) {
#pragma unroll
          for (int i = 0; i < 16; ++i) K0a[i] = K0b[i] = 0.f;
        }
      }
#undef M64_STEP
      lds_barrier();
    }
    Ra = K2a; Rb = K2b; K2a = K1a; K2b = K1b; K1a = K0a; K1b = K0b;
  }
#pragma unroll
  for (int i = 0; i < 16; ++i) retire_elem(Ra, 0, i);
  retire_flush(0, d1 - 1);
#pragma unroll
  for (int i = 0; i < 16; ++i) retire_elem(Rb, 1, i);
  retire_flush(1, d1 - 1);

  if (stats) {
    lds_barrier();
    float* red = reinterpret_cast<float*>(smem);
    const float a = ssum + __shfl_xor(ssum, 32, 64), q2 = qsum + __shfl_xor(qsum, 32, 64);
    if (lane < 32) { red[(wave * 2 + 0) * 32 + r] = a; red[(wave * 2 + 1) * 32 + r] = q2; }
    lds_barrier();
    if (tid < 64) {
      const int which = tid >> 5, c = tid & 31;
      float tt = 0.f;
#pragma unroll
      for (int wv = 0; wv < 4; ++wv) tt += red[(wv * 2 + which) * 32 + c];
      stats[((int64_t)bid.x * 2 + which) * Cout + n0 + c] = tt;
    }
  }
}

struct MarchCfg { int tilesH, tilesW, dsegs, dlen, nblk, fw; };

inline bool march_enabled() {
  return fplx_knob(FPLX_K_MARCH) != 0;
}

inline MarchCfg march_cfg(int n, int d, int h, int w, int cin, int cout) {
  MarchCfg c;
  int fh = cin >= 64 ? MG64::FH : MG::FH;
  c.fw = 32;
  if (cin >= 64) {
    const int kfw = (int)fplx_knob(FPLX_K_MARCH64_FW);
    const int64_t a32 = (int64_t)((h + 7) / 8) * 8 * ((w + 31) / 32) * 32;
    const int64_t a16 = (int64_t)((h + 15) / 16) * 16 * ((w + 15) / 16) * 16;
    if ((kfw == 0 && a16 < a32) || kfw == 16) { c.fw = 16; fh = 16; }
  }
  c.tilesH = (h + fh - 1) / fh;
  c.tilesW = (w + c.fw - 1) / c.fw;
  const int64_t tiles = (int64_t)n * c.tilesH * c.tilesW * (cout / 32);
  double best = 1e30;
  int best_ds = 1;
  for (int ds = 1; ds <= d; ++ds) {
    const int dl = (d + ds - 1) / ds;
    if (dl < 4 && ds > 1) break;
    const int segs = (d + dl - 1) / dl;
    if (d - (segs - 1) * dl < 2 && d >= 2) continue;
    const int64_t rounds = (tiles * segs + 255) / 256;
    const double cost = (double)rounds * (dl + 2 + 1.5);
    if (cost < best - 1e-9) { best = cost; best_ds = segs; }
  }
  {
    const int e = (int)fplx_knob(FPLX_K_MARCH_DS);
    if (e > 0) best_ds = e;
  }
  c.dlen = (d + best_ds - 1) / best_ds;
  c.dsegs = (d + c.dlen - 1) / c.dlen;
  c.nblk = n * c.tilesH * c.tilesW * c.dsegs;
  return c;
}

}

extern "C" int fplx_march_ok(int n, int d, int h, int w, int cin, int cout) {
  if (!march_enabled() || cout % 32 != 0 || d < 4 || w < 64) return 0;
  if (cin == 32) return h >= 16;
  if (cin == 64) return h >= 8 && (int64_t)h * w * 64 * 2 < (int64_t)1 << 31;
  if (cin == 128) {
    const int k128 = (int)fplx_knob(FPLX_K_MARCH128);
    return k128 && h >= 8 && (int64_t)h * w * 128 * 2 < (int64_t)1 << 31;
  }
  return 0;
}

extern "C" int fplx_march_variant(int n, int d, int h, int w, int cin, int cout) {
  if (cin == 32)
    return (fplx_knob(FPLX_K_MARCH32_V2) && h % MG2::FH == 0 && w % MG2::FW == 0 && (int64_t)d * h * w * cin * 2 <= ((int64_t)1 << 30)) ? 2 : 0;
  return march_cfg(n, d, h, w, cin, cout).fw;
}

extern "C" int fplx_march_rows(int n, int d, int h, int w, int cin, int cout) {
  return march_cfg(n, d, h, w, cin, cout).nblk;
}

extern "C" int fplx_march_conv3d_fwd_act(const void* x, int64_t ldx, const void* wp, const float* bias, void* y, int64_t ldy,
                                         int n, int d, int h, int w, int cin, int cout, float* stats, hipStream_t st,
                                         const void* x1, void* y1, int twod, const float* slope, int nmod0) {
  if (ldy % 8 != 0 || ((uintptr_t)y % 16) != 0 || ldx % 8 != 0 || ((uintptr_t)x % 16) != 0 || ((uintptr_t)wp % 16) != 0 ||
      ((uintptr_t)x1 % 16) != 0 || ((uintptr_t)y1 % 16) != 0)
    return 0;
  const MarchCfg c = march_cfg(n, d, h, w, cin, cout);
  dim3 grid(c.nblk, cout / 32);
  if (cin >= 64) {
    if (y1 || (cin == 128 && x1)) return 0;
    const bool lw64 = twod && fplx_knob(FPLX_K_MARCH64_LW) != 0 && (int64_t)h * w * ldx * 2 < ((int64_t)1 << 30);
    auto launch = [&](auto kernel, int threads, int lds) {
      fplx_launch(kernel, grid, threads, lds, st, (const bf16_t*)x, ldx, (const bf16_t*)wp, bias, (bf16_t*)y, ldy, n, d, h, w, cout,
                  slope ? nullptr : stats, c.tilesH, c.tilesW, c.dsegs, c.dlen, (const bf16_t*)x1, fplx_xcd_on(), slope,
                  slope ? nmod0 : 0);
    };
#define M64_KERNEL(K_, G_, TWOD_)                                                                                    \
  (cin == 128 ? (slope ? K_<G_, TWOD_, 4, true> : K_<G_, TWOD_, 4>) : (slope ? K_<G_, TWOD_, 2, true> : K_<G_, TWOD_, 2>))
#define M64_FOOTPRINT(G_)                                                                                            \
  do {                                                                                                              \
    if (lw64) launch(M64_KERNEL(conv_fwd_march64_lw, G_, true), 512, G_::LDS);                                       \
    else if (twod) launch(M64_KERNEL(conv_fwd_march64, G_, true), G_::THREADS, G_::LDS);                             \
    else launch(M64_KERNEL(conv_fwd_march64, G_, false), G_::THREADS, G_::LDS);                                      \
  } while (0)
    if (c.fw == 16) M64_FOOTPRINT(MG64T<16>); else M64_FOOTPRINT(MG64);
#undef M64_FOOTPRINT
#undef M64_KERNEL
    const int rc64 = fplx_check_launch("march64_conv3d_fwd");
    return rc64 < 0 ? rc64 : 1;
  }
  if (x1) return 0;
  {
    const int kv2 = (int)fplx_knob(FPLX_K_MARCH32_V2);
    if (kv2 && !twod && h % MG2::FH == 0 && w % MG2::FW == 0 && (int64_t)d * h * w * ldx * 2 <= ((int64_t)1 << 30)) {
      auto launch = [&](auto kernel, auto... slope_arg) {
        fplx_launch(kernel, grid, MG2::THREADS, MG2::LDS, st, (const bf16_t*)x, ldx, (const bf16_t*)wp, bias, (bf16_t*)y, ldy, n, d, h,
                    w, cout, slope ? nullptr : stats, c.tilesH, c.tilesW, c.dsegs, c.dlen, (bf16_t*)y1, y1 ? cout / 64 : cout / 32,
                    fplx_xcd_on(), slope_arg...);
      };
      if (slope) launch(conv_fwd_march32v3<false, 1, true>, slope);
      else if (stats) { if (kv2 == 3) launch(conv_fwd_march32v3<true, 1>, nullptr); else launch(conv_fwd_march32v2<true>); }
      else { if (kv2 >= 3) launch(conv_fwd_march32v3<false, 1>, nullptr); else launch(conv_fwd_march32v2<false>); }
      const int rc2 = fplx_check_launch("march32v2_conv3d_fwd");
      return rc2 < 0 ? rc2 : 1;
    }
  }
  const auto k = slope ? (twod ? conv_fwd_march32<true, true> : conv_fwd_march32<false, true>)
                       : (twod ? conv_fwd_march32<true> : conv_fwd_march32<false>);
  fplx_launch(k, grid, MG::THREADS, MG::LDS, st, (const bf16_t*)x, ldx, (const bf16_t*)wp, bias, (bf16_t*)y, ldy, n, d, h, w, cout,
              slope ? nullptr : stats, c.tilesH, c.tilesW, c.dsegs, c.dlen, (bf16_t*)y1, y1 ? cout / 64 : cout / 32, fplx_xcd_on(), slope);
  const int rc = fplx_check_launch("march_conv3d_fwd");
  return rc < 0 ? rc : 1;
}

extern "C" int fplx_march_conv3d_fwd(const void* x, int64_t ldx, const void* wp, const float* bias, void* y, int64_t ldy,
                                     int n, int d, int h, int w, int cin, int cout, float* stats, hipStream_t st,
                                     const void* x1, void* y1, int twod) {
  return fplx_march_conv3d_fwd_act(x, ldx, wp, bias, y, ldy, n, d, h, w, cin, cout, stats, st, x1, y1, twod, nullptr, 0);
}
```

### fpl-plus_amd/csrc/gfx950.h

```cpp
#pragma once
#include "common.h"

typedef __attribute__((ext_vector_type(8))) __bf16 bf16x8;
typedef __attribute__((ext_vector_type(4))) __bf16 bf16x4;
typedef __attribute__((ext_vector_type(16))) float f32x16;
typedef __attribute__((ext_vector_type(4))) float f32x4;
typedef __attribute__((ext_vector_type(2))) float f32x2;
typedef __attribute__((ext_vector_type(4))) unsigned int u32x4;
typedef __attribute__((ext_vector_type(2))) unsigned int u32x2;
typedef __attribute__((address_space(3))) bf16x4 lds_bf16x4;

template <class T> __device__ __forceinline__ void opaque_v(T& x) { asm volatile("" : "+v"(x)); }
template <class T> __device__ __forceinline__ void opaque_s(T& x) { asm volatile("" : "+s"(x)); }
template <class T> __device__ __forceinline__ void opaque_v(T& x, T& y) { asm volatile("" : "+v"(x), "+v"(y)); }

__device__ __forceinline__ void wait_vmcnt0() { asm volatile("s_waitcnt vmcnt(0)" ::: "memory"); }
template <int N> __device__ __forceinline__ void wait_vmcnt() { asm volatile("s_waitcnt vmcnt(%0)" :: "n"(N) : "memory"); }
__device__ __forceinline__ void wait_vmcnt_upto8(int n) {
  if (n == 1) wait_vmcnt<1>();
  else if (n == 2) wait_vmcnt<2>();
  else if (n == 3) wait_vmcnt<3>();
  else if (n == 4) wait_vmcnt<4>();
  else if (n == 5) wait_vmcnt<5>();
  else if (n == 6) wait_vmcnt<6>();
  else if (n == 7) wait_vmcnt<7>();
  else if (n == 8) wait_vmcnt<8>();
  else wait_vmcnt0();
}
__device__ __forceinline__ void lds_barrier() { asm volatile("s_waitcnt lgkmcnt(0)\n\ts_barrier" ::: "memory"); }

__device__ __forceinline__ unsigned lds_addr(const void* p) {
  return __builtin_amdgcn_readfirstlane((unsigned)(size_t)((__attribute__((address_space(3))) char*)p));
}

__device__ __forceinline__ bf16x8 tr_splice(bf16x4 lo, bf16x4 hi) {
  bf16x8 r;
  r[0] = lo[0]; r[1] = lo[1]; r[2] = lo[2]; r[3] = lo[3];
  r[4] = hi[0]; r[5] = hi[1]; r[6] = hi[2]; r[7] = hi[3];
  return r;
}
#pragma clang diagnostic push
#pragma clang diagnostic ignored "-Wint-to-pointer-cast"
template <class A> __device__ __forceinline__ bf16x8 tr_frag(A base_lo) {
  return tr_splice(__builtin_amdgcn_ds_read_tr16_b64_v4bf16((lds_bf16x4*)(base_lo)),
                   __builtin_amdgcn_ds_read_tr16_b64_v4bf16((lds_bf16x4*)(base_lo + 4 * 64)));
}
#pragma clang diagnostic pop

struct BufferBase {
  unsigned lo, hi;
  __device__ __forceinline__ BufferBase(uint64_t a)
      : lo(__builtin_amdgcn_readfirstlane((unsigned)a)), hi(__builtin_amdgcn_readfirstlane((unsigned)(a >> 32) & 0xFFFFu)) {}
  __device__ __forceinline__ BufferBase(const void* p) : BufferBase((uint64_t)(size_t)p) {}
};
__device__ __forceinline__ u32x4 buffer_rsrc(BufferBase base, unsigned bytes) {
  u32x4 r;
  r[0] = base.lo;
  r[1] = base.hi;
  r[2] = __builtin_amdgcn_readfirstlane(bytes);
  r[3] = 0x00020000u;
  return r;
}

__device__ __forceinline__ void lds_dma_buffer(u32x4 rsrc, unsigned lane_off, unsigned scalar_off, unsigned lds) {
  unsigned keep;
  asm volatile("s_mov_b32 %0, m0\n\ts_mov_b32 m0, %4\n\ts_nop 0\n\tbuffer_load_dwordx4 %1, %2, %3 offen lds\n\ts_mov_b32 m0, %0"
               : "=&s"(keep) : "v"(lane_off), "s"(rsrc), "s"(scalar_off), "s"(lds) : "memory");
}
__device__ __forceinline__ void lds_dma_global(const void* src, unsigned lds) {
  unsigned keep;
  asm volatile("s_mov_b32 %0, m0\n\ts_mov_b32 m0, %2\n\ts_nop 0\n\tglobal_load_lds_dwordx4 %1, off\n\ts_mov_b32 m0, %0"
               : "=&s"(keep) : "v"(src), "s"(lds) : "memory");
}

__device__ __forceinline__ void global_store_16(void* dst, u32x4 v) {
  asm volatile("global_store_dwordx4 %0, %1, off\n\ts_nop 1" :: "v"(dst), "v"(v) : "memory");
}
```

### include/fplx.h

```cpp
#ifndef FPLX_H
#define FPLX_H

#include <stddef.h>
#include <stdint.h>

#ifdef __cplusplus
extern "C" {
#endif
#pragma GCC visibility push(default)

typedef void* fplx_stream_t;

enum { FPLX_F32 = 0, FPLX_BF16 = 1 };

enum {
  FPLX_OK = 0,
  FPLX_E_BADSHAPE = -1,
  FPLX_E_BADDTYPE = -2,
  FPLX_E_WORKSPACE = -3,
  FPLX_E_HIP = -4,
  FPLX_E_NULL = -5
};

int fplx_version(void);
int fplx_last_error(char* buf, size_t n);
int fplx_num_partials(int64_t voxels);

enum {
  FPLX_KERNEL_GENERIC = 0, FPLX_KERNEL_DIRECT = 1, FPLX_KERNEL_TILE = 2, FPLX_KERNEL_STREAM = 3, FPLX_KERNEL_MARCH = 4,
  FPLX_KERNEL_BRICK = 5, FPLX_KERNEL_STEM = 6, FPLX_KERNEL_OUTCONV = 7
};
int fplx_set_tuning(const char* key, int64_t value);
int fplx_get_tuning(const char* key, int64_t* value);
int fplx_tuning_key(int index, char* buf, size_t n);
int fplx_conv3d_plan_query(int n, int d, int h, int w, int cin, int cout, int kd, int kh, int kw, int x_dt, int y_dt,
                           int* kernel, int* geometry, int* ksplit, int* stats_rows);

int fplx_pack_conv_weight(const float* w, void* wf, void* wb, int cout, int cin, int kd, int kh, int kw,
                          int dt, fplx_stream_t stream);
int fplx_pack_conv_weights_batched(int n, const float* const* w, void* const* wf, void* const* wb, const int* cout,
                                   const int* cin, int dt, float* const* stamp, int verify, fplx_stream_t stream);
int fplx_pack_weights_multi(int n, const int* kind, const float* const* w, void* const* wf, void* const* wb, const int* a,
                            const int* b, const int* taps, const int* dt, fplx_stream_t stream);
int fplx_pack_deconv_weight(const float* w, void* wf, void* wb, int cin, int cout, int dt,
                            fplx_stream_t stream);

int fplx_conv3d_stats_rows(int n, int d, int h, int w, int cin, int cout, int kd, int kh, int kw, int x_dt, int y_dt);
size_t fplx_conv3d_fwd_ws_bytes(int n, int d, int h, int w, int cin, int cout, int kd, int kh, int kw, int x_dt, int y_dt);
int fplx_conv3d_fwd(const void* x, int x_dt, int64_t sn, int64_t sd, int64_t sh, int64_t sw, int64_t sc,
                    const void* wp, const float* bias,
                    void* y, int y_dt, int64_t yn, int64_t yd, int64_t yh, int64_t yw, int64_t yc,
                    int n, int d, int h, int w, int cin, int cout, int kd, int kh, int kw,
                    float* stats, void* ws, size_t ws_bytes, fplx_stream_t stream);

size_t fplx_conv3d_wgrad_ws_bytes(int n, int d, int h, int w, int cin, int cout, int kd, int kh, int kw);
int fplx_conv3d_wgrad(const void* x, int x_dt, int64_t sn, int64_t sd, int64_t sh, int64_t sw, int64_t sc,
                      const void* dy, int dy_dt, int64_t yn, int64_t yd, int64_t yh, int64_t yw, int64_t yc,
                      float* dw, float* db, int n, int d, int h, int w, int cin, int cout,
                      int kd, int kh, int kw, void* ws, size_t ws_bytes, fplx_stream_t stream);

int fplx_stem_wgrad_bn(const float* x, const void* y, int64_t ldy, const void* dout, int64_t ldd, const float* mean,
                       const float* rstd, const float* scale, const float* shift, const float* slope, const float* coef,
                       float* dw, int n, int d, int h, int w, int cin, int cout, void* ws, size_t ws_bytes, fplx_stream_t stream);

int fplx_conv3d_cat2_ok(int n, int d, int h, int w, int cin, int cout);
int fplx_conv3d_fwd_cat2(const void* x0, const void* x1, int64_t ldx, const void* wp, const float* bias, void* y,
                         int64_t ldy, int n, int d, int h, int w, int cin, int cout, float* stats,
                         fplx_stream_t stream);
int fplx_conv3d_dgrad_split2(const void* dy, int64_t ldy, const void* wb, void* dx0, void* dx1, int64_t ldx, int n,
                             int d, int h, int w, int cin, int cout, fplx_stream_t stream);
int fplx_conv3d_wgrad_cat2(const void* x0, const void* x1, int64_t ldx, const void* dy, int64_t ldy, float* dw, int n,
                           int d, int h, int w, int cin, int cout, void* ws, size_t ws_bytes, fplx_stream_t stream);

int fplx_conv3d_fwd_act_ok(int n, int d, int h, int w, int cin, int cout, int mid, int cat2);
int fplx_conv3d_fwd_act(const void* x0, const void* x1, int64_t ldx, const void* wp, const float* bias,
                        const float* prelu_slope, void* y, int64_t ldy, int n, int d, int h, int w, int cin, int cout,
                        int mid, int n_x0, void* ws, size_t ws_bytes, fplx_stream_t stream);

int fplx_deconv2_fwd(const void* x, int64_t ldx, const void* wf, const float* bias, void* y, int64_t ldy,
                     int n, int d, int h, int w, int cin, int cout, int dt, fplx_stream_t stream);
int fplx_deconv2_dgrad(const void* dy, int64_t ldy, const void* wb, void* dx, int64_t ldx,
                       int n, int d, int h, int w, int cin, int cout, int dt, fplx_stream_t stream);
size_t fplx_deconv2_wgrad_ws_bytes(int n, int d, int h, int w, int cin, int cout);
int fplx_deconv2_wgrad(const void* x, int64_t ldx, const void* dy, int64_t ldy, float* dw, float* db,
                       int n, int d, int h, int w, int cin, int cout, int dt,
                       void* ws, size_t ws_bytes, fplx_stream_t stream);

int fplx_pack_conv2d_weight(const float* w, void* wf, void* wb, int cout, int cin, int dt, fplx_stream_t stream);
int fplx_conv2d_stats_rows(int n, int d, int h, int w, int cin, int cout, int x_dt, int y_dt);
size_t fplx_conv2d_fwd_ws_bytes(int n, int d, int h, int w, int cin, int cout, int x_dt, int y_dt);
int fplx_conv2d_fwd(const void* x, int x_dt, int64_t sn, int64_t sd, int64_t sh, int64_t sw, int64_t sc,
                    const void* wp, const float* bias, void* y, int y_dt, int64_t yn, int64_t yd, int64_t yh,
                    int64_t yw, int64_t yc, int n, int d, int h, int w, int cin, int cout,
                    float* stats, void* ws, size_t ws_bytes, fplx_stream_t stream);
int fplx_conv2d_fwd_cat2(const void* x0, const void* x1, int64_t ldx, const void* wp, const float* bias, void* y,
                         int64_t ldy, int n, int d, int h, int w, int cin, int cout, float* stats,
                         fplx_stream_t stream);
int fplx_conv2d_dgrad_split2(const void* dy, int64_t ldy, const void* wb, void* dx0, void* dx1, int64_t ldx, int n,
                             int d, int h, int w, int cin, int cout, fplx_stream_t stream);
size_t fplx_conv2d_wgrad_ws_bytes(int n, int d, int h, int w, int cin, int cout);
int fplx_conv2d_wgrad(const void* x, int x_dt, int64_t sn, int64_t sd, int64_t sh, int64_t sw, int64_t sc,
                      const void* dy, int dy_dt, int64_t yn, int64_t yd, int64_t yh, int64_t yw, int64_t yc,
                      float* dw, float* db, int n, int d, int h, int w, int cin, int cout,
                      void* ws, size_t ws_bytes, fplx_stream_t stream);
int fplx_conv2d_wgrad_cat2(const void* x0, const void* x1, int64_t ldx, const void* dy, int64_t ldy, float* dw, int n,
                           int d, int h, int w, int cin, int cout, void* ws, size_t ws_bytes, fplx_stream_t stream);
int fplx_maxpool122_fwd(const void* x, int64_t ldx, void* y, int64_t ldy, int n, int d, int h, int w, int c,
                        int dt, fplx_stream_t stream);
int fplx_maxpool122_bwd(const void* x, int64_t ldx, const void* dy, int64_t ldy, const void* dskip, int64_t lds,
                        void* dx, int64_t ldo, int n, int d, int h, int w, int c, int dt, fplx_stream_t stream);
int fplx_pack_deconv122_weight(const float* w, void* wf, void* wb, int cin, int cout, int dt, fplx_stream_t stream);
int fplx_deconv122_fwd(const void* x, int64_t ldx, const void* wf, const float* bias, void* y, int64_t ldy,
                       int n, int d, int h, int w, int cin, int cout, int dt, fplx_stream_t stream);
int fplx_deconv122_dgrad(const void* dy, int64_t ldy, const void* wb, void* dx, int64_t ldx,
                         int n, int d, int h, int w, int cin, int cout, int dt, fplx_stream_t stream);
size_t fplx_deconv122_wgrad_ws_bytes(int n, int d, int h, int w, int cin, int cout);
int fplx_deconv122_wgrad(const void* x, int64_t ldx, const void* dy, int64_t ldy, float* dw, float* db,
                         int n, int d, int h, int w, int cin, int cout, int dt,
                         void* ws, size_t ws_bytes, fplx_stream_t stream);

int fplx_bn_train_finalize(const float* stats, int rows, int c, int64_t count,
                           const float* gamma, const float* beta, float* running_mean, float* running_var,
                           int64_t* num_batches_tracked, float momentum, float eps,
                           float* mean, float* rstd, float* scale, float* shift, fplx_stream_t stream);
int fplx_channel_stats(const void* x, int64_t ldx, int64_t voxels, int c, int dt, float* stats,
                       fplx_stream_t stream);
int fplx_bn_eval_prepare(const float* gamma, const float* beta, const float* running_mean,
                         const float* running_var, float eps, int c, float* scale, float* shift,
                         fplx_stream_t stream);
int fplx_bn_act_fwd(const void* y, int64_t ldy, void* out, int64_t ldo, const float* scale, const float* shift,
                    const float* slope, float p, uint64_t seed, uint32_t stream_id,
                    int64_t voxels, int c, int dt, fplx_stream_t stream);
int fplx_bn_act_bwd_reduce(const void* y, int64_t ldy, const void* dout, int64_t ldd,
                           const float* mean, const float* rstd, const float* scale, const float* shift,
                           const float* slope, float p, uint64_t seed, uint32_t stream_id,
                           int64_t voxels, int c, int dt, float* part, fplx_stream_t stream);
int fplx_bn_act_bwd_finalize(const float* part, int rows, int c, int64_t count, int train,
                             float* dgamma, float* dbeta, float* dslope, float* coef, fplx_stream_t stream);
int fplx_bn_act_bwd_apply(const void* y, int64_t ldy, const void* dout, int64_t ldd, void* dy, int64_t ldo,
                          const float* mean, const float* rstd, const float* scale, const float* shift,
                          const float* slope, const float* coef, float p, uint64_t seed, uint32_t stream_id,
                          int64_t voxels, int c, int dt, fplx_stream_t stream);

int fplx_maxpool2_fwd(const void* x, int64_t ldx, void* y, int64_t ldy, int n, int d, int h, int w, int c,
                      int dt, fplx_stream_t stream);
int fplx_maxpool2_bwd(const void* x, int64_t ldx, const void* dy, int64_t ldy, const void* dskip, int64_t lds,
                      void* dx, int64_t ldo, int n, int d, int h, int w, int c, int dt, fplx_stream_t stream);

int fplx_bn_pool_fused_ok(int c, int dt);
int fplx_bn_act_pool_fwd(const void* y, int64_t ldy, void* out, int64_t ldo, void* pooled, int64_t ldp, const float* scale,
                         const float* shift, const float* slope, int n, int d, int h, int w, int c, int dt, int pd,
                         fplx_stream_t stream);
int fplx_pool_bwd_bn_reduce(const void* y, int64_t ldy, const void* dy, int64_t lddy, const void* dskip, int64_t lds, void* dx,
                            int64_t ldo, const float* mean, const float* rstd, const float* scale, const float* shift,
                            const float* slope, int n, int d, int h, int w, int c, int dt, int pd, float* part,
                            fplx_stream_t stream);

int fplx_outconv_bn_rows(int n, int d, int h, int w, int c0, int ncls);
int fplx_outconv_fwd_bn(const void* y, int64_t ldy, const float* scale, const float* shift, const float* prelu_slope, void* a,
                        int64_t lda, const float* wf, const float* bias, float* logits, int n, int d, int h, int w, int c0,
                        int ncls, fplx_stream_t stream);
int fplx_outconv_dgrad_bn_reduce(const float* dlogits, const void* wb, const void* y, int64_t ldy, const float* mean,
                                 const float* rstd, const float* scale, const float* shift, const float* prelu_slope,
                                 float* part, int n, int d, int h, int w, int c0, int ncls, fplx_stream_t stream);
int fplx_outconv_dgrad_bn_apply(const float* dlogits, const void* wb, const void* y, int64_t ldy, const float* mean,
                                const float* rstd, const float* scale, const float* shift, const float* prelu_slope,
                                const float* coef, void* dy, int64_t lddy, int n, int d, int h, int w, int c0, int ncls,
                                fplx_stream_t stream);
size_t fplx_outconv_wgrad_bn_ws_bytes(int n, int d, int h, int w, int c0, int ncls);
int fplx_outconv_wgrad_bn(const void* y, int64_t ldy, const float* scale, const float* shift, const float* prelu_slope,
                          const float* dlogits, float* dw, float* db, int n, int d, int h, int w, int c0, int ncls, void* ws,
                          size_t ws_bytes, fplx_stream_t stream);

int fplx_upsample2_fwd(const void* x, int64_t ldx, void* y, int64_t ldy, int n, int d, int h, int w, int c, int dt, int sd,
                       fplx_stream_t stream);
int fplx_upsample2_bwd(const void* dy, int64_t ldy, void* dx, int64_t ldx, int n, int d, int h, int w, int c, int dt, int sd,
                       fplx_stream_t stream);

int fplx_head_fwd(const void* a, int64_t lda, int dt, const float* w, const float* bias, float* logits, int n, int64_t v, int c,
                  int ncls, fplx_stream_t stream);
int fplx_head_dgrad(const float* dlogits, const float* w, void* da, int64_t lda, int dt, int n, int64_t v, int c, int ncls,
                    int accumulate, fplx_stream_t stream);
size_t fplx_head_wgrad_ws_bytes(int n, int64_t v, int c, int ncls);
int fplx_head_wgrad(const void* a, int64_t lda, int dt, const float* dlogits, float* dw, float* db, int n, int64_t v, int c,
                    int ncls, void* ws, size_t ws_bytes, fplx_stream_t stream);
int fplx_interp_fwd(const float* x, float* y, int64_t nc, int d, int h, int w, int f, fplx_stream_t stream);
int fplx_interp_bwd(const float* dy, float* dx, int64_t nc, int d, int h, int w, int f, fplx_stream_t stream);

#define FPLX_LOSS_K(C) (6 * (C) + 3)
int fplx_loss_rows(int64_t voxels_per_sample);
int fplx_seg_loss_fwd(const float* logits, const float* label, const float* pixel_weight,
                      const float* image_weight, int n, int c, int64_t voxels_per_sample,
                      float w_dice, float w_ce, float w_dice_img, float w_entropy, int softmax,
                      float* part, float* out, float* coef, fplx_stream_t stream);
int fplx_seg_loss_sums(const float* logits, const float* label, const float* pixel_weight, int n, int c,
                       int64_t voxels_per_sample, int softmax, float* part, double* sums, double* totals,
                       fplx_stream_t stream);
int fplx_seg_loss_from_sums(const double* sums, const double* totals, const float* image_weight, int n, int n_global, int c,
                            int64_t voxels_per_sample, int has_pixel_weight, float w_dice, float w_ce, float w_dice_img,
                            float w_entropy, float* out, float* coef, fplx_stream_t stream);
int fplx_seg_loss_bwd(const float* logits, const float* label, const float* pixel_weight,
                      const float* coef, const float* gscale, int n, int c, int64_t voxels_per_sample,
                      float w_dice, float w_ce, float w_dice_img, float w_entropy, int softmax,
                      float* dlogits, fplx_stream_t stream);

#define FPLX_LOSS_EXT_K(C) (10 * (C) + 7)
#define FPLX_LOSS_EXT_NCFG(C) (18 + (C))
#define FPLX_LOSS_EXT_NOUT(C) (4 + (C) + 7)
#define FPLX_LOSS_EXT_NCOEF(N, C) ((N) * (C) * 2 + 2 + 4 * (C) + 4)
int fplx_seg_loss_ext_fwd(const float* logits, const float* label, const float* pixel_weight, const float* image_weight,
                          int n, int c, int64_t voxels_per_sample, const float* cfg, int softmax, float* part, float* out,
                          float* coef, fplx_stream_t stream);
int fplx_seg_loss_ext_sums(const float* logits, const float* label, const float* pixel_weight, int n, int c,
                           int64_t voxels_per_sample, const float* cfg, int softmax, float* part, double* sums,
                           double* totals, fplx_stream_t stream);
int fplx_seg_loss_ext_from_sums(const double* sums, const double* totals, const float* image_weight, int n, int n_global,
                                int c, int64_t voxels_per_sample, int has_pixel_weight, const float* cfg, float* out,
                                float* coef, fplx_stream_t stream);
int fplx_seg_loss_ext_bwd(const float* logits, const float* label, const float* pixel_weight, const float* coef,
                          const float* gscale, int n, int c, int64_t voxels_per_sample, const float* cfg, int softmax,
                          float* dlogits, fplx_stream_t stream);

int fplx_adam_step(float* p, const float* g, float* m, float* v, int64_t n, float lr, float beta1, float beta2,
                   float eps, float weight_decay, int step, float grad_scale, fplx_stream_t stream);
int fplx_adam_pack_ok(int cout, int cin);
int fplx_adam_pack_step(float* p, const float* g, float* m, float* v, int64_t n, float lr, float beta1, float beta2, float eps,
                        float weight_decay, int step, float grad_scale, int nl, const int64_t* off, const int* cout,
                        const int* cin, void* const* wf, void* const* wb, float* const* stamp, fplx_stream_t stream);
enum { FPLX_OPT_SGD = 0, FPLX_OPT_ADADELTA, FPLX_OPT_ADAGRAD, FPLX_OPT_ADAMAX, FPLX_OPT_ASGD, FPLX_OPT_RMSPROP, FPLX_OPT_RPROP,
       FPLX_OPT_ADAM, FPLX_OPT_COUNT };
int fplx_optim_step(int kind, float* p, const float* g, float* s0, float* s1, int64_t n, const float* hp, int nhp, int step,
                    float grad_scale, fplx_stream_t stream);
int fplx_optim_pack_step(int kind, float* p, const float* g, float* s0, float* s1, int64_t n, const float* hp, int nhp, int step,
                         float grad_scale, int nl, const int64_t* off, const int* cout, const int* cin, void* const* wf,
                         void* const* wb, float* const* stamp, fplx_stream_t stream);

int fplx_mc_filter(const float* logits, int t, int c, int64_t v, float thr, uint8_t* hards,
                   float* mean_out, float* unc_out, double* part, double* out, fplx_stream_t stream);
int fplx_hard_label(const float* logits, int n, int c, int64_t v, uint8_t* out, fplx_stream_t stream);
int fplx_pixel_weight(const uint8_t* a, const uint8_t* b, int64_t v, int apply_set_weight, float image_weight,
                      float* out, fplx_stream_t stream);

size_t fplx_normalize_ws_bytes(void);
int fplx_normalize_mean_std(const float* x, float* y, int64_t n, const float* mean_std, void* ws, size_t ws_bytes,
                            float* out_mean_std, fplx_stream_t stream);
int fplx_normalize_positive(const float* x, const float* noise, float* y, int64_t n, void* ws, size_t ws_bytes,
                            float* out_mean_std, fplx_stream_t stream);
int fplx_pad_reflect(const void* x, void* y, int elem_bytes, int c, int d, int h, int w, int lo_d, int lo_h, int lo_w,
                     int od, int oh, int ow, fplx_stream_t stream);
int fplx_crop_flip(const void* x, void* y, int elem_bytes, int c, int d, int h, int w, int cd, int ch, int cw, int od,
                   int oh, int ow, int flip_mask, fplx_stream_t stream);
int fplx_label_bbox(const unsigned char* label, int c, int d, int h, int w, const int* mask_labels, int nmask, int* out9,
                    fplx_stream_t stream);
int fplx_label_to_probability(const unsigned char* label, float* prob, int class_num, int64_t voxels,
                              fplx_stream_t stream);
int fplx_set_weight(float* pixel_weight, int64_t n, float image_weight, fplx_stream_t stream);

int fplx_nonzero_bbox(const float* x, int c, int d, int h, int w, int* out9, fplx_stream_t stream);
int fplx_label_lut(const uint8_t* in, uint8_t* out, int64_t n, const uint8_t* lut256, fplx_stream_t stream);
int fplx_partial_label_to_probability(const uint8_t* label, float* prob, float* weight, int class_num, int64_t voxels,
                                      int* max_label, fplx_stream_t stream);
int fplx_paste_roi(const void* sub, void* out, int elem_bytes, int c, int sd, int sh, int sw, int od, int oh, int ow,
                   int lo_d, int lo_h, int lo_w, fplx_stream_t stream);

int fplx_resample_affine(const void* x, void* y, int elem_bytes, int order, int c, int d, int h, int w, int od, int oh,
                         int ow, const double* matrix9, const double* offset3, fplx_stream_t stream);

int fplx_spline_prefilter(const float* x, double* coef, int c, int d, int h, int w, int order, fplx_stream_t stream);
int fplx_resample_spline(const double* coef, float* y, int c, int d, int h, int w, int od, int oh, int ow,
                         const double* matrix9, const double* offset3, int order, fplx_stream_t stream);

#define FPLX_EDT_MAX_EXTENT 620
#define FPLX_EDT_WS_BYTES(n, voxels) ((size_t)2 * (size_t)(n) * (size_t)(voxels) * 4)
int fplx_edt_squared(const uint8_t* mask, int n, int d, int h, int w, int ndim, const double* sampling3, const uint8_t* phantom,
                     double* sq, int* idx, int* ws, size_t ws_bytes, fplx_stream_t stream);
int fplx_edt_pass(double* g, int n, int d, int h, int w, int axis, double sampling, fplx_stream_t stream);
int fplx_edt_finish(const double* sq_a, const double* sq_b, double* out, int64_t count, fplx_stream_t stream);

int fplx_sw_extract(const float* image, int n, int c, int d, int h, int w, const int* starts_d, int nd, const int* starts_h,
                    int nh, const int* starts_w, int nw, int wd, int wh, int ww, const int* flips, int nflips, float* patches,
                    fplx_stream_t stream);
int fplx_sw_merge(const float* patches, int n, int c, int d, int h, int w, const int* starts_d, int nd, const int* starts_h,
                  int nh, const int* starts_w, int nw, int wd, int wh, int ww, const int* flips, int nflips, float* out,
                  fplx_stream_t stream);
int fplx_sw_merge_mc(const float* patches, int passes, int chunk, int n, int c, int d, int h, int w, const int* starts_d, int nd,
                     const int* starts_h, int nh, const int* starts_w, int nw, int wd, int wh, int ww, const int* flips,
                     int nflips, float* out, fplx_stream_t stream);

int fplx_overlap_counts(const unsigned char* seg, const unsigned char* gt, int64_t n, const int* labels, int nlabels,
                        int fuse, unsigned long long* out, fplx_stream_t stream);

int fplx_surface_edge_points(const unsigned char* img, int d, int h, int w, unsigned char* edge, fplx_stream_t stream);
int fplx_surface_min_dist(const int* query_zyx, int64_t nq, const int* seed_zyx, int64_t ns, float sz, float sy, float sx,
                          float* out, fplx_stream_t stream);

#define FPLX_CC_LABEL_WS_BYTES(voxels) ((size_t)320 * 4)
#define FPLX_KLC_WS_BYTES(voxels) (((size_t)320 + 2 * (size_t)(voxels)) * 4)
int fplx_cc_label(const uint8_t* seg, int d, int h, int w, int per_class, int* labels, int* ws, size_t ws_bytes,
                  fplx_stream_t stream);
int fplx_keep_largest_component(const uint8_t* seg, int d, int h, int w, int per_class, uint8_t* out, int* ws,
                                size_t ws_bytes, fplx_stream_t stream);

int fplx_channel_minmax(const float* x, int64_t n, float lo, int use_lo, float hi, int use_hi, void* ws, size_t ws_bytes,
                        float* out4, fplx_stream_t stream);
size_t fplx_select_ws_bytes(void);
int fplx_select_kth(const float* x, int64_t n, const int64_t* ranks, int nranks, float* out, void* ws, size_t ws_bytes,
                    fplx_stream_t stream);
int fplx_clip_affine(const float* x, float* y, int64_t n, float v0, float v1, float a, float b, fplx_stream_t stream);
int fplx_clip_affine_dev(const float* x, float* y, int64_t n, const float* v0, const float* v1, const float* a,
                         const float* hi, fplx_stream_t stream);
int fplx_threshold_replace(const float* x, float* y, int64_t n, float t_lo, float r_lo, int use_lo, float t_hi, float r_hi,
                           int use_hi, fplx_stream_t stream);
int fplx_normalize_range(const float* x, const float* noise, float* y, int64_t n, float v0, int use_v0, float v1, int use_v1,
                         void* ws, size_t ws_bytes, float* out_mean_std, fplx_stream_t stream);
int fplx_gamma(const float* x, float* y, int64_t n, const float* vmin, const float* vmax, float gamma, fplx_stream_t stream);
int fplx_add_noise_f64(const float* x, const double* noise, float* y, int64_t n, fplx_stream_t stream);
int fplx_add_noise_philox(const float* x, float* y, int64_t n, uint64_t seed, uint32_t stream_id, double mean, double sigma,
                          double* out_uniforms, fplx_stream_t stream);

int fplx_ssl_perturb(const float* x, const float* noise, float* y, int64_t n, int reps, float sigma, float clip, uint64_t seed,
                     uint32_t stream_id, fplx_stream_t stream);
int fplx_ssl_consistency_fwd(const float* student, const float* teacher, const float* mc, int t, int n, int c,
                             int64_t voxels_per_sample, float thr, int softmax, uint8_t* mask, float* part, double* out,
                             fplx_stream_t stream);
int fplx_ssl_consistency_bwd(const float* student, const float* teacher, const uint8_t* mask, const double* out,
                             const float* gscale, int n, int c, int64_t voxels_per_sample, int t, int softmax, float* dstudent,
                             fplx_stream_t stream);
int fplx_ssl_entropy_fwd(const float* logits, int n, int c, int64_t voxels_per_sample, int softmax, float* part, double* out,
                         fplx_stream_t stream);
int fplx_ssl_entropy_bwd(const float* logits, const float* gscale, int n, int c, int64_t voxels_per_sample, int softmax,
                         float* dlogits, fplx_stream_t stream);
int fplx_ema_step(float* ema, const float* p, int64_t n, float alpha, fplx_stream_t stream);
int fplx_ssl_pyramid_fwd(const float* const* logits, int k, int n, int c, int64_t voxels_per_sample, float* part, double* out,
                         fplx_stream_t stream);
int fplx_ssl_pyramid_bwd(const float* const* logits, const double* out, const float* gscale, int k, int n, int c,
                         int64_t voxels_per_sample, float* const* dlogits, fplx_stream_t stream);
int fplx_ssl_pseudo_onehot(const float* const* logits, int k, int n, int c, int64_t voxels_per_sample, float* const* onehot,
                           fplx_stream_t stream);

int fplx_wsl_gatedcrf_fwd(const float* logits, const float* image, int n, int c, int ci, int d, int h, int w, const float* desc,
                          int nk, int radius, int softmax, float* kp, float* part, double* out, fplx_stream_t stream);
int fplx_wsl_gatedcrf_bwd(const float* logits, const float* kp, const float* gscale, int n, int c, int d, int h, int w,
                          int softmax, float* dlogits, fplx_stream_t stream);
int fplx_wsl_tv_fwd(const float* logits, int n, int c, int d, int h, int w, int softmax, int32_t* count, void* ws,
                    size_t ws_bytes, float* part, double* out, fplx_stream_t stream);
int fplx_wsl_tv_bwd(const float* logits, const int32_t* count, const float* gscale, int n, int c, int d, int h, int w,
                    int softmax, float* dlogits, fplx_stream_t stream);
int fplx_wsl_mumford_shah_fwd(const float* logits, const float* image, int n, int c, int ci, int d, int h, int w, int penalty,
                              float lambda, int softmax, float* cen, float* part, double* out, fplx_stream_t stream);
int fplx_wsl_mumford_shah_bwd(const float* logits, const float* image, const float* cen, const float* gscale, int n, int c,
                              int ci, int d, int h, int w, int penalty, float lambda, int softmax, float* dlogits,
                              fplx_stream_t stream);

enum { FPLX_NLL_RANK = 0, FPLX_NLL_BELOW = 1 };
int fplx_nll_ce_rows(int64_t voxels_per_sample);
int fplx_nll_voxel_ce_fwd(const float* const* logits, int k, const float* label, int n, int c, int64_t voxels_per_sample,
                          float* const* loss, float* part, fplx_stream_t stream);
size_t fplx_nll_mask_ws_bytes(void);
int fplx_nll_select_mask(const float* loss, int64_t n, int mode, int64_t num_remb, float w, const float* sk, const float* smax,
                         uint8_t* mask, void* ws, size_t ws_bytes, fplx_stream_t stream);
size_t fplx_nll_select_ws_bytes(void);
int fplx_nll_select_fwd(const float* const* loss, const uint8_t* const* mask, const int* uses, int k, int64_t n,
                        const float* ce_part, int64_t ce_rows, double* out, void* ws, size_t ws_bytes, fplx_stream_t stream);
int fplx_nll_select_bwd(const float* const* logits, const float* label, const uint8_t* const* mask, const int* uses, int k,
                        const double* out, const float* gscale, float wj, int n, int c, int64_t voxels_per_sample,
                        float* const* dlogits, fplx_stream_t stream);

#pragma GCC visibility pop
#ifdef __cplusplus
}
#endif
#endif
```

Measured before the change: 248.4 volumes/s.

## Chain consecutive depth segments per block in march conv forward kernels

Lets each march forward block (march32v2/v3, 3D march64 with 64 input channels) process a chain of consecutive work units instead of one. Weights and bias are loaded into LDS once per block, and adjacent depth segments merge into one longer march that skips repeated halo slab loads. The chain length comes from the device's CU count, so the grid roughly matches one wave of blocks. Per-unit BN stats rows are flushed mid-march into an extra 1 KB of LDS. The trade-offs are fewer blocks and less parallelism, more LDS per block, and more complex stats bookkeeping.

```diff
diff --git a/fpl-plus_amd/csrc/common.h b/fpl-plus_amd/csrc/common.h
--- a/fpl-plus_amd/csrc/common.h
+++ b/fpl-plus_amd/csrc/common.h
@@ -270,6 +270,8 @@
   X(MARCH, "march", 1)                           \
   X(MARCH64_FW, "march64_fw", 0)                                \
   X(MARCH_DS, "march_ds", 0)                                       \
+  X(MARCH_CHAIN, "march_chain", 3)          \
+  X(MARCH_CHAIN_BLOCKS, "march_chain_blocks", 0)  \
   X(MARCH128, "march128", 1)                                                                                           \
   X(MARCH64_LW, "march64_lw", 1)            \
   X(MARCH32_V2, "march32_v2", 4)              \
diff --git a/fpl-plus_amd/csrc/conv_march.hip b/fpl-plus_amd/csrc/conv_march.hip
--- a/fpl-plus_amd/csrc/conv_march.hip
+++ b/fpl-plus_amd/csrc/conv_march.hip
@@ -284,7 +284,7 @@
 conv_fwd_march32v2(const bf16_t* __restrict__ x, int64_t ldx, const bf16_t* __restrict__ wp,
                    const float* __restrict__ bias, bf16_t* __restrict__ y, int64_t ldy, int N, int D, int H, int W,
                    int Cout, float* __restrict__ stats, int tilesH, int tilesW, int dsegs, int dlen,
-                   bf16_t* __restrict__ y1, int ysplit, int xcd) {
+                   bf16_t* __restrict__ y1, int ysplit, int xcd, int nunits, int chain) {
   using G = MG2;
   extern __shared__ __attribute__((aligned(16))) char smem[];
   char* slabs = smem;
@@ -292,17 +292,28 @@
   float* bias_s = reinterpret_cast<float*>(wbuf + G::W_BYTES);
   const int tid = threadIdx.x, lane = tid & 63;
   const int wave = __builtin_amdgcn_readfirstlane(tid >> 6);
+  const FplxBlock bid = fplx_xcd_block(xcd);
+  const int n0 = bid.y * 32;
+  const int u_begin = __builtin_amdgcn_readfirstlane(bid.x * chain);
+  const int u_end = u_begin + chain < nunits ? u_begin + chain : nunits;
+  for (int j = wave; j < 27 * 32 * G::CH / 64; j += G::WAVES) {
+    const int i = j * 64 + lane;
+    const int row = i >> 2, c = (i & 3) ^ G::swz(row);
+    lds_dma_global(wp + ((int64_t)(row >> 5) * Cout + n0 + (row & 31)) * G::CIN + c * 8, lds_addr(wbuf + j * 1024));
+  }
+  if (tid < 32) bias_s[tid] = bias ? bias[n0 + tid] : 0.f;
+  for (int u = u_begin; u < u_end;) {
+  const int lane = fresh_lane(), tid = wave * 64 + lane;
   const int r = lane & 31, khalf = lane >> 5;
-  const FplxBlock bid = fplx_xcd_block(xcd);
-  int b = bid.x;
+  int b = u;
   const int seg = b % dsegs; b /= dsegs;
   const int tw = b % tilesW; b /= tilesW;
   const int th = b % tilesH; b /= tilesH;
   const int n = __builtin_amdgcn_readfirstlane(b);
+  const int nseg = dsegs - seg < u_end - u ? dsegs - seg : u_end - u;
   const int h0 = __builtin_amdgcn_readfirstlane(th * G::FH), w0 = __builtin_amdgcn_readfirstlane(tw * G::FW);
   const int d0 = __builtin_amdgcn_readfirstlane(seg * dlen);
-  const int d1 = (d0 + dlen < D) ? d0 + dlen : D;
-  const int n0 = bid.y * 32;
+  const int d1 = (d0 + nseg * dlen < D) ? d0 + nseg * dlen : D;
 
   constexpr int NPIECE = G::NPIECE;
   unsigned* voff_s = reinterpret_cast<unsigned*>(smem + 2 * G::SLAB_BYTES + G::W_BYTES + 32 * 4 + G::WAVES * 2 * G::STAGE_BYTES);
@@ -333,28 +344,40 @@
   };
 
   f32x16 S[4][4];
+  float z0 = 0.f;
+  opaque_v(z0);
 #pragma unroll
   for (int a = 0; a < 4; ++a)
 #pragma unroll
     for (int m = 0; m < 4; ++m)
 #pragma unroll
-      for (int i = 0; i < 16; ++i) S[a][m][i] = 0.f;
+      for (int i = 0; i < 16; ++i) S[a][m][i] = z0;
 
   __syncthreads();
   const int sbase = d0 - 1;
 #pragma unroll
   for (int k = 0; k < NPIECE; ++k) slab_piece(sbase, k, voff_s[k * G::THREADS + tid]);
-  for (int j = wave; j < 27 * 32 * G::CH / 64; j += G::WAVES) {
-    const int i = j * 64 + lane;
-    const int row = i >> 2, c = (i & 3) ^ G::swz(row);
-    lds_dma_global(wp + ((int64_t)(row >> 5) * Cout + n0 + (row & 31)) * G::CIN + c * 8, lds_addr(wbuf + j * 1024));
-  }
-  if (tid < 32) bias_s[tid] = bias ? bias[n0 + tid] : 0.f;
   wait_vmcnt0();
   lds_barrier();
 
   const float bv = bias_s[r];
   float ssum = 0.f, qsum = 0.f;
+  auto stats_flush = [&](int row) {
+    float* red = reinterpret_cast<float*>(smem + G::LDS);
+    lds_barrier();
+    const float a = ssum + __shfl_xor(ssum, 32, 64), q2 = qsum + __shfl_xor(qsum, 32, 64);
+    const int fl = fresh_lane();
+    if (fl < 32) { red[(wave * 2 + 0) * 32 + fl] = a; red[(wave * 2 + 1) * 32 + fl] = q2; }
+    lds_barrier();
+    if (wave == 0) {
+      const int which = fl >> 5, c = fl & 31;
+      float tt = 0.f;
+#pragma unroll
+      for (int wv = 0; wv < 4; ++wv) tt += red[(wv * 2 + which) * 32 + c];
+      stats[((int64_t)row * 2 + which) * Cout + n0 + c] = tt;
+    }
+    ssum = 0.f; qsum = 0.f;
+  };
   char* stg = reinterpret_cast<char*>(bias_s + 32) + wave * 2 * G::STAGE_BYTES;
   const unsigned ldy2 = (unsigned)ldy * 2u;
   bf16_t* ysel = bid.y >= ysplit ? y1 + (bid.y - ysplit) * 32 : y + n0;
@@ -491,17 +514,29 @@
   const long long st_begin = __builtin_amdgcn_s_memtime();
   const long long st_rbegin = __builtin_amdgcn_s_memrealtime();
 #endif
-  int t = 0;
+  int t = 0, urow = u, tflush = dlen + 3;
+  auto between = [&]() {
+    if (STATS) {
+      if (t == 3) { ssum = 0.f; qsum = 0.f; }
+      if (t == tflush) {
+        if (stats) stats_flush(urow);
+        ++urow; tflush += dlen;
+      }
+    }
+  };
   for (;;) {
     step(C0{}, t); ++t;
     if (t >= nsteps) break;
+    between();
     step(C1{}, t); ++t;
     if (t >= nsteps) break;
+    between();
     step(C2{}, t); ++t;
     if (t >= nsteps) break;
-    if (STATS && t == 3) { ssum = 0.f; qsum = 0.f; }
+    between();
     step(C3{}, t); ++t;
     if (t >= nsteps) break;
+    between();
   }
 #ifdef FPLX_STAMP
   if (lane == 0) {
@@ -523,19 +558,8 @@
     default: drain(C3{}); break;
   }
 
-  if (STATS && stats) {
-    lds_barrier();
-    float* red = reinterpret_cast<float*>(smem);
-    const float a = ssum + __shfl_xor(ssum, 32, 64), q2 = qsum + __shfl_xor(qsum, 32, 64);
-    if (lane < 32) { red[(wave * 2 + 0) * 32 + r] = a; red[(wave * 2 + 1) * 32 + r] = q2; }
-    lds_barrier();
-    if (tid < 64) {
-      const int which = tid >> 5, c = tid & 31;
-      float tt = 0.f;
-#pragma unroll
-      for (int wv = 0; wv < 4; ++wv) tt += red[(wv * 2 + which) * 32 + c];
-      stats[((int64_t)bid.x * 2 + which) * Cout + n0 + c] = tt;
-    }
+  if (STATS && stats) stats_flush(urow);
+  u += nseg;
   }
 }
 
@@ -544,7 +568,8 @@
 conv_fwd_march32v3(const bf16_t* __restrict__ x, int64_t ldx, const bf16_t* __restrict__ wp,
                    const float* __restrict__ bias, bf16_t* __restrict__ y, int64_t ldy, int N, int D, int H, int W,
                    int Cout, float* __restrict__ stats, int tilesH, int tilesW, int dsegs, int dlen,
-                   bf16_t* __restrict__ y1, int ysplit, int xcd, const float* __restrict__ slope_p = nullptr) {
+                   bf16_t* __restrict__ y1, int ysplit, int xcd, int nunits, int chain,
+                   const float* __restrict__ slope_p = nullptr) {
   using G = MG2;
   extern __shared__ __attribute__((aligned(16))) char smem[];
   char* slabs = smem;
@@ -552,19 +577,32 @@
   float* bias_s = reinterpret_cast<float*>(wbuf + G::W_BYTES);
   const int tid = threadIdx.x, lane = tid & 63;
   const int wave = __builtin_amdgcn_readfirstlane(tid >> 6);
+  const FplxBlock bid = fplx_xcd_block(xcd);
+  const int n0 = bid.y * 32;
+  constexpr bool CHAINS = !STATS;
+  const int u_begin = __builtin_amdgcn_readfirstlane(CHAINS ? bid.x * chain : bid.x);
+  const int u_end = !CHAINS ? u_begin + 1 : (u_begin + chain < nunits ? u_begin + chain : nunits);
+
+  auto wswz = [](int row) { const int q = (row >> 2) & 3; return (4 - q) & 3; };
+  for (int j = wave; j < 27 * 32 * G::CH / 64; j += G::WAVES) {
+    const int i = j * 64 + lane;
+    const int row = i >> 2, c = (i & 3) ^ wswz(row);
+    lds_dma_global(wp + ((int64_t)(row >> 5) * Cout + n0 + (row & 31)) * G::CIN + c * 8, lds_addr(wbuf + j * 1024));
+  }
+  if (tid < 32) bias_s[tid] = bias ? bias[n0 + tid] : 0.f;
+  for (int u = u_begin; u < u_end;) {
+  const int lane = fresh_lane(), tid = wave * 64 + lane;
   const int r16 = lane & 15, kg = lane >> 4;
-  const FplxBlock bid = fplx_xcd_block(xcd);
-  int b = bid.x;
+  int b = u;
   const int seg = b % dsegs; b /= dsegs;
   const int tw = b % tilesW; b /= tilesW;
   const int th = b % tilesH; b /= tilesH;
   const int n = __builtin_amdgcn_readfirstlane(b);
+  const int nseg = !CHAINS ? 1 : (dsegs - seg < u_end - u ? dsegs - seg : u_end - u);
   const int h0 = __builtin_amdgcn_readfirstlane(th * G::FH), w0 = __builtin_amdgcn_readfirstlane(tw * G::FW);
   const int d0 = __builtin_amdgcn_readfirstlane(seg * dlen);
-  const int d1 = (d0 + dlen < D) ? d0 + dlen : D;
-  const int n0 = bid.y * 32;
-
-  auto wswz = [](int row) { const int q = (row >> 2) & 3; return (4 - q) & 3; };
+  const int d1 = (d0 + nseg * dlen < D) ? d0 + nseg * dlen : D;
+
   auto aswz = [](int vox) { return ASWZ ? ((vox >> 2) & 1) << 1 : (vox >> 2) & 3; };
   constexpr int NPIECE = G::NPIECE;
   unsigned* voff_s = reinterpret_cast<unsigned*>(smem + 2 * G::SLAB_BYTES + G::W_BYTES + 32 * 4 + G::WAVES * 2 * G::STAGE_BYTES);
@@ -595,6 +633,8 @@
   };
 
   f32x4 S[4][4][4];
+  float z0 = 0.f;
+  opaque_v(z0);
 #pragma unroll
   for (int a = 0; a < 4; ++a)
 #pragma unroll
@@ -602,23 +642,39 @@
 #pragma unroll
       for (int q = 0; q < 4; ++q)
 #pragma unroll
-        for (int i = 0; i < 4; ++i) S[a][m][q][i] = 0.f;
+        for (int i = 0; i < 4; ++i) S[a][m][q][i] = z0;
 
   __syncthreads();
   const int sbase = d0 - 1;
 #pragma unroll
   for (int k = 0; k < NPIECE; ++k) slab_piece(sbase, k, voff_s[k * G::THREADS + tid]);
-  for (int j = wave; j < 27 * 32 * G::CH / 64; j += G::WAVES) {
-    const int i = j * 64 + lane;
-    const int row = i >> 2, c = (i & 3) ^ wswz(row);
-    lds_dma_global(wp + ((int64_t)(row >> 5) * Cout + n0 + (row & 31)) * G::CIN + c * 8, lds_addr(wbuf + j * 1024));
-  }
-  if (tid < 32) bias_s[tid] = bias ? bias[n0 + tid] : 0.f;
   wait_vmcnt0();
   lds_barrier();
 
   const float bv0 = bias_s[r16], bv1 = bias_s[16 + r16];
   float ssum0 = 0.f, qsum0 = 0.f, ssum1 = 0.f, qsum1 = 0.f;
+  auto stats_flush = [&](int row) {
+    float* red = reinterpret_cast<float*>(smem + G::LDS);
+    lds_barrier();
+    float a0 = ssum0, a1 = ssum1, q0 = qsum0, q1 = qsum1;
+    a0 += __shfl_xor(a0, 16, 64); a0 += __shfl_xor(a0, 32, 64);
+    a1 += __shfl_xor(a1, 16, 64); a1 += __shfl_xor(a1, 32, 64);
+    q0 += __shfl_xor(q0, 16, 64); q0 += __shfl_xor(q0, 32, 64);
+    q1 += __shfl_xor(q1, 16, 64); q1 += __shfl_xor(q1, 32, 64);
+    if (lane < 16) {
+      red[(wave * 2 + 0) * 32 + r16] = a0; red[(wave * 2 + 0) * 32 + 16 + r16] = a1;
+      red[(wave * 2 + 1) * 32 + r16] = q0; red[(wave * 2 + 1) * 32 + 16 + r16] = q1;
+    }
+    lds_barrier();
+    if (tid < 64) {
+      const int which = tid >> 5, c = tid & 31;
+      float tt = 0.f;
+#pragma unroll
+      for (int wv = 0; wv < 4; ++wv) tt += red[(wv * 2 + which) * 32 + c];
+      stats[((int64_t)row * 2 + which) * Cout + n0 + c] = tt;
+    }
+    ssum0 = qsum0 = ssum1 = qsum1 = 0.f;
+  };
   char* stg = reinterpret_cast<char*>(bias_s + 32) + wave * 2 * G::STAGE_BYTES;
   const unsigned ldy2 = (unsigned)ldy * 2u;
   bf16_t* ysel = bid.y >= ysplit ? y1 + (bid.y - ysplit) * 32 : y + n0;
@@ -766,16 +822,23 @@
   const long long st_rbegin = __builtin_amdgcn_s_memrealtime();
 #endif
   int t = 0;
+  const int urow = u;
+  auto between = [&]() {
+    if (STATS && t == 3) { ssum0 = qsum0 = ssum1 = qsum1 = 0.f; }
+  };
   for (;;) {
     step(C0{}, t); ++t;
     if (t >= nsteps) break;
+    between();
     step(C1{}, t); ++t;
     if (t >= nsteps) break;
+    between();
     step(C2{}, t); ++t;
     if (t >= nsteps) break;
-    if (STATS && t == 3) { ssum0 = qsum0 = ssum1 = qsum1 = 0.f; }
+    between();
     step(C3{}, t); ++t;
     if (t >= nsteps) break;
+    between();
   }
 #ifdef FPLX_STAMP
   if (lane == 0) {
@@ -797,26 +860,8 @@
     default: drain(C3{}); break;
   }
 
-  if (STATS && stats) {
-    lds_barrier();
-    float* red = reinterpret_cast<float*>(smem);
-    float a0 = ssum0, a1 = ssum1, q0 = qsum0, q1 = qsum1;
-    a0 += __shfl_xor(a0, 16, 64); a0 += __shfl_xor(a0, 32, 64);
-    a1 += __shfl_xor(a1, 16, 64); a1 += __shfl_xor(a1, 32, 64);
-    q0 += __shfl_xor(q0, 16, 64); q0 += __shfl_xor(q0, 32, 64);
-    q1 += __shfl_xor(q1, 16, 64); q1 += __shfl_xor(q1, 32, 64);
-    if (lane < 16) {
-      red[(wave * 2 + 0) * 32 + r16] = a0; red[(wave * 2 + 0) * 32 + 16 + r16] = a1;
-      red[(wave * 2 + 1) * 32 + r16] = q0; red[(wave * 2 + 1) * 32 + 16 + r16] = q1;
-    }
-    lds_barrier();
-    if (tid < 64) {
-      const int which = tid >> 5, c = tid & 31;
-      float tt = 0.f;
-#pragma unroll
-      for (int wv = 0; wv < 4; ++wv) tt += red[(wv * 2 + which) * 32 + c];
-      stats[((int64_t)bid.x * 2 + which) * Cout + n0 + c] = tt;
-    }
+  if (STATS && stats) stats_flush(urow);
+  u += nseg;
   }
 }
 
@@ -888,7 +933,8 @@
 conv_fwd_march64(const bf16_t* __restrict__ x, int64_t ldx, const bf16_t* __restrict__ wp,
                  const float* __restrict__ bias, bf16_t* __restrict__ y, int64_t ldy, int N, int D, int H, int W,
                  int Cout, float* __restrict__ stats, int tilesH, int tilesW, int dsegs, int dlen,
-                 const bf16_t* __restrict__ x1, int xcd, const float* __restrict__ slope_p = nullptr, int nmod0 = 0) {
+                 const bf16_t* __restrict__ x1, int xcd, const float* __restrict__ slope_p, int nmod0, int nunits,
+                 int chain) {
   extern __shared__ __attribute__((aligned(16))) char smem[];
   char* slabs = smem;
   char* wbuf = smem + 2 * G::SLAB_BYTES;
@@ -897,15 +943,29 @@
   const int wave = __builtin_amdgcn_readfirstlane(tid >> 6);
   const int r = lane & 31, khalf = lane >> 5;
   const FplxBlock bid = fplx_xcd_block(xcd);
-  int b = bid.x;
+  const int n0 = bid.y * 32;
+  constexpr bool CHAINS = !TWOD && NQ == 2;
+  const int u_begin = __builtin_amdgcn_readfirstlane(CHAINS ? bid.x * chain : bid.x);
+  const int u_end = !CHAINS ? u_begin + 1 : (u_begin + chain < nunits ? u_begin + chain : nunits);
+  if constexpr (NQ == 2) {
+    for (int j = wave; j < 2 * 27 * 32 * G::CH / 64; j += 4) {
+      const int i = j * 64 + lane;
+      const int hf = i / (27 * 32 * G::CH), ii = i % (27 * 32 * G::CH);
+      const int row = ii >> 2, c = (ii & 3) ^ G::swz(row);
+      lds_dma_global(wp + ((int64_t)(row >> 5) * Cout + n0 + (row & 31)) * 64 + hf * 32 + c * 8, lds_addr(wbuf + j * 1024));
+    }
+  }
+  if (tid < 32) bias_s[tid] = bias ? bias[n0 + tid] : 0.f;
+  for (int u = u_begin; u < u_end;) {
+  int b = u;
   const int seg = b % dsegs; b /= dsegs;
   const int tw = b % tilesW; b /= tilesW;
   const int th = b % tilesH; b /= tilesH;
   const int n = __builtin_amdgcn_readfirstlane(b);
+  const int nseg = !CHAINS ? 1 : (dsegs - seg < u_end - u ? dsegs - seg : u_end - u);
   const int h0 = __builtin_amdgcn_readfirstlane(th * G::FH), w0 = __builtin_amdgcn_readfirstlane(tw * G::FW);
   const int d0 = __builtin_amdgcn_readfirstlane(seg * dlen);
-  const int d1 = (d0 + dlen < D) ? d0 + dlen : D;
-  const int n0 = bid.y * 32;
+  const int d1 = (d0 + nseg * dlen < D) ? d0 + nseg * dlen : D;
 
   constexpr int NPIECE = G::NPIECE;
   int soff[NPIECE];
@@ -944,22 +1004,29 @@
 #pragma unroll
     for (int k = 0; k < NPIECE; ++k) { slab_piece(sbase, 0, k); }
   }
-  if constexpr (NQ == 2) {
-    for (int j = wave; j < 2 * 27 * 32 * G::CH / 64; j += 4) {
-      const int i = j * 64 + lane;
-      const int hf = i / (27 * 32 * G::CH), ii = i % (27 * 32 * G::CH);
-      const int row = ii >> 2, c = (ii & 3) ^ G::swz(row);
-      lds_dma_global(wp + ((int64_t)(row >> 5) * Cout + n0 + (row & 31)) * 64 + hf * 32 + c * 8, lds_addr(wbuf + j * 1024));
-    }
-  } else {
+  if constexpr (NQ != 2) {
     for (int j = wave; j < 54; j += 4) w_piece(0, j);
   }
-  if (tid < 32) bias_s[tid] = bias ? bias[n0 + tid] : 0.f;
   wait_vmcnt0();
   lds_barrier();
 
   const float bv = bias_s[r];
   float ssum = 0.f, qsum = 0.f;
+  auto stats_flush = [&](int row) {
+    float* red = reinterpret_cast<float*>(smem + G::LDS);
+    lds_barrier();
+    const float a = ssum + __shfl_xor(ssum, 32, 64), q2 = qsum + __shfl_xor(qsum, 32, 64);
+    if (lane < 32) { red[(wave * 2 + 0) * 32 + r] = a; red[(wave * 2 + 1) * 32 + r] = q2; }
+    lds_barrier();
+    if (tid < 64) {
+      const int which = tid >> 5, c = tid & 31;
+      float tt = 0.f;
+#pragma unroll
+      for (int wv = 0; wv < 4; ++wv) tt += red[(wv * 2 + which) * 32 + c];
+      stats[((int64_t)row * 2 + which) * Cout + n0 + c] = tt;
+    }
+    ssum = 0.f; qsum = 0.f;
+  };
   char* stg = reinterpret_cast<char*>(bias_s + 32) + wave * G::STAGE_BYTES;
   char* stg_w = stg + (4 * khalf) * 64 + r * 2;
   const char* stg_r = stg + lane * 16;
@@ -1010,6 +1077,7 @@
 
   const int nd = d1 - d0;
   const int nsteps = TWOD ? nd + 1 : nd + 2;
+  int urow = u, tflush = dlen + 2;
   for (int t = 0; t < nsteps; ++t) {
     const int s = sbase + t;
     const bool live = TWOD ? t < nd : (s >= 0 && s < D);
@@ -1069,6 +1137,12 @@
       lds_barrier();
     }
     Ra = K2a; Rb = K2b; K2a = K1a; K2b = K1b; K1a = K0a; K1b = K0b;
+    if constexpr (CHAINS) {
+      if (t == tflush) {
+        if (stats) stats_flush(urow);
+        ++urow; tflush += dlen;
+      }
+    }
   }
 #pragma unroll
   for (int i = 0; i < 16; ++i) retire_elem(Ra, 0, i);
@@ -1077,19 +1151,8 @@
   for (int i = 0; i < 16; ++i) retire_elem(Rb, 1, i);
   retire_flush(1, d1 - 1);
 
-  if (stats) {
-    lds_barrier();
-    float* red = reinterpret_cast<float*>(smem);
-    const float a = ssum + __shfl_xor(ssum, 32, 64), q2 = qsum + __shfl_xor(qsum, 32, 64);
-    if (lane < 32) { red[(wave * 2 + 0) * 32 + r] = a; red[(wave * 2 + 1) * 32 + r] = q2; }
-    lds_barrier();
-    if (tid < 64) {
-      const int which = tid >> 5, c = tid & 31;
-      float tt = 0.f;
-#pragma unroll
-      for (int wv = 0; wv < 4; ++wv) tt += red[(wv * 2 + which) * 32 + c];
-      stats[((int64_t)bid.x * 2 + which) * Cout + n0 + c] = tt;
-    }
+  if (stats) stats_flush(urow);
+  u += nseg;
   }
 }
 
@@ -1355,6 +1418,40 @@
   return c;
 }
 
+inline int march_device_cus() {
+  static int cus[64];
+  int dev = 0;
+  if (hipGetDevice(&dev) != hipSuccess || dev < 0 || dev >= 64) return 0;
+  int c = __atomic_load_n(&cus[dev], __ATOMIC_RELAXED);
+  if (c <= 0) {
+    if (hipDeviceGetAttribute(&c, hipDeviceAttributeMultiprocessorCount, dev) != hipSuccess || c <= 0) return 0;
+    __atomic_store_n(&cus[dev], c, __ATOMIC_RELAXED);
+  }
+  return c;
+}
+
+struct MarchChain { int blocks, chain; };
+inline int march_chain(const MarchCfg& c, int groups, bool fwd, MarchChain* out) {
+  out->blocks = c.nblk; out->chain = 1;
+  if (!(fplx_knob(FPLX_K_MARCH_CHAIN) & (fwd ? 1 : 2))) return FPLX_OK;
+  const int kb = (int)fplx_knob(FPLX_K_MARCH_CHAIN_BLOCKS);
+  int cus = groups;
+  if (kb > 0) cus = kb > c.nblk ? groups * c.nblk : groups * kb;
+  else if ((cus = march_device_cus()) <= 0) return fplx_fail(FPLX_E_HIP, "march_conv3d_fwd: no compute-unit count for the device");
+  return fplx_march_chain_plan(c.nblk, groups, cus, &out->blocks, &out->chain);
+}
+
+}
+
+extern "C" int fplx_march_chain_plan(int units, int groups, int cus, int* blocks, int* chain) {
+  FPLX_REQUIRE(units > 0 && groups > 0 && cus > 0 && blocks && chain, FPLX_E_BADSHAPE, "march_chain_plan: bad arguments");
+  int bg = cus / groups;
+  if (bg < 1) bg = 1;
+  if (bg > units) bg = units;
+  const int l = (units + bg - 1) / bg;
+  *chain = l;
+  *blocks = (units + l - 1) / l;
+  return FPLX_OK;
 }
 
 extern "C" int fplx_march_ok(int n, int d, int h, int w, int cin, int cout) {
@@ -1389,18 +1486,24 @@
   if (cin >= 64) {
     if (y1 || (cin == 128 && x1)) return 0;
     const bool lw64 = twod && fplx_knob(FPLX_K_MARCH64_LW) != 0 && (int64_t)h * w * ldx * 2 < ((int64_t)1 << 30);
-    auto launch = [&](auto kernel, int threads, int lds) {
+    MarchChain ch = {c.nblk, 1};
+    if (!twod && cin == 64) {
+      const int rcc = march_chain(c, cout / 32, stats || slope, &ch);
+      if (rcc < 0) return rcc;
+      grid.x = ch.blocks;
+    }
+    auto launch = [&](auto kernel, int threads, int lds, auto... chain_args) {
       fplx_launch(kernel, grid, threads, lds, st, (const bf16_t*)x, ldx, (const bf16_t*)wp, bias, (bf16_t*)y, ldy, n, d, h, w, cout,
                   slope ? nullptr : stats, c.tilesH, c.tilesW, c.dsegs, c.dlen, (const bf16_t*)x1, fplx_xcd_on(), slope,
-                  slope ? nmod0 : 0);
+                  slope ? nmod0 : 0, chain_args...);
     };
 #define M64_KERNEL(K_, G_, TWOD_)                                                                                    \
   (cin == 128 ? (slope ? K_<G_, TWOD_, 4, true> : K_<G_, TWOD_, 4>) : (slope ? K_<G_, TWOD_, 2, true> : K_<G_, TWOD_, 2>))
 #define M64_FOOTPRINT(G_)                                                                                            \
   do {                                                                                                              \
     if (lw64) launch(M64_KERNEL(conv_fwd_march64_lw, G_, true), 512, G_::LDS);                                       \
-    else if (twod) launch(M64_KERNEL(conv_fwd_march64, G_, true), G_::THREADS, G_::LDS);                             \
-    else launch(M64_KERNEL(conv_fwd_march64, G_, false), G_::THREADS, G_::LDS);                                      \
+    else if (twod) launch(M64_KERNEL(conv_fwd_march64, G_, true), G_::THREADS, G_::LDS + 1024, c.nblk, 1);           \
+    else launch(M64_KERNEL(conv_fwd_march64, G_, false), G_::THREADS, G_::LDS + 1024, c.nblk, ch.chain);             \
   } while (0)
     if (c.fw == 16) M64_FOOTPRINT(MG64T<16>); else M64_FOOTPRINT(MG64);
 #undef M64_FOOTPRINT
@@ -1412,10 +1515,16 @@
   {
     const int kv2 = (int)fplx_knob(FPLX_K_MARCH32_V2);
     if (kv2 && !twod && h % MG2::FH == 0 && w % MG2::FW == 0 && (int64_t)d * h * w * ldx * 2 <= ((int64_t)1 << 30)) {
+      MarchChain ch = {c.nblk, 1};
+      if (!(stats && !slope && kv2 == 3)) {
+        const int rcc = march_chain(c, cout / 32, stats || slope, &ch);
+        if (rcc < 0) return rcc;
+      }
+      grid.x = ch.blocks;
       auto launch = [&](auto kernel, auto... slope_arg) {
-        fplx_launch(kernel, grid, MG2::THREADS, MG2::LDS, st, (const bf16_t*)x, ldx, (const bf16_t*)wp, bias, (bf16_t*)y, ldy, n, d, h,
-                    w, cout, slope ? nullptr : stats, c.tilesH, c.tilesW, c.dsegs, c.dlen, (bf16_t*)y1, y1 ? cout / 64 : cout / 32,
-                    fplx_xcd_on(), slope_arg...);
+        fplx_launch(kernel, grid, MG2::THREADS, MG2::LDS + 1024, st, (const bf16_t*)x, ldx, (const bf16_t*)wp, bias, (bf16_t*)y, ldy,
+                    n, d, h, w, cout, slope ? nullptr : stats, c.tilesH, c.tilesW, c.dsegs, c.dlen, (bf16_t*)y1,
+                    y1 ? cout / 64 : cout / 32, fplx_xcd_on(), c.nblk, ch.chain, slope_arg...);
       };
       if (slope) launch(conv_fwd_march32v3<false, 1, true>, slope);
       else if (stats) { if (kv2 == 3) launch(conv_fwd_march32v3<true, 1>, nullptr); else launch(conv_fwd_march32v2<true>); }
diff --git a/fpl-plus_amd/csrc/gfx950.h b/fpl-plus_amd/csrc/gfx950.h
--- a/fpl-plus_amd/csrc/gfx950.h
+++ b/fpl-plus_amd/csrc/gfx950.h
@@ -12,6 +12,11 @@
 
 template <class T> __device__ __forceinline__ void opaque_v(T& x) { asm volatile("" : "+v"(x)); }
 template <class T> __device__ __forceinline__ void opaque_s(T& x) { asm volatile("" : "+s"(x)); }
+__device__ __forceinline__ int fresh_lane() {
+  unsigned z = 0;
+  asm volatile("" : "+v"(z));
+  return (int)__builtin_amdgcn_mbcnt_hi(~0u, __builtin_amdgcn_mbcnt_lo(~0u, z));
+}
 template <class T> __device__ __forceinline__ void opaque_v(T& x, T& y) { asm volatile("" : "+v"(x), "+v"(y)); }
 
 __device__ __forceinline__ void wait_vmcnt0() { asm volatile("s_waitcnt vmcnt(0)" ::: "memory"); }
diff --git a/include/fplx.h b/include/fplx.h
--- a/include/fplx.h
+++ b/include/fplx.h
@@ -35,6 +35,7 @@
 int fplx_tuning_key(int index, char* buf, size_t n);
 int fplx_conv3d_plan_query(int n, int d, int h, int w, int cin, int cout, int kd, int kh, int kw, int x_dt, int y_dt,
                            int* kernel, int* geometry, int* ksplit, int* stats_rows);
+int fplx_march_chain_plan(int units, int groups, int cus, int* blocks, int* chain);
 
 int fplx_pack_conv_weight(const float* w, void* wf, void* wb, int cout, int cin, int kd, int kh, int kw,
                           int dt, fplx_stream_t stream);
```

Measured after the change: 248.3 volumes/s. About the same (-0.0%).
